# yixuan/LBFGSpp

Hardware: NVIDIA B200
Metric: lbfgs_iterations_per_sec (higher is better)
Workload: dtype f64

## Files before the change

### lbfgspp_b200/csrc/device_utils.cuh

```cuda
#pragma once

#include <cuda_runtime.h>
#include <stdint.h>

namespace lb {

constexpr int kThreads = 256;
constexpr int kMaxRed = 8;
constexpr int kMaxBlocks = 148 * 8;

template <class T> struct Pack { T v[4]; };

enum class Hint { Stream, Keep, Plain };

template <Hint H> __device__ __forceinline__ Pack<double> ld_pack(const double* p)
{
    Pack<double> r;
    if (H == Hint::Stream)
        asm("ld.global.L1::no_allocate.L2::evict_first.v4.f64 {%0,%1,%2,%3}, [%4];"
                     : "=d"(r.v[0]), "=d"(r.v[1]), "=d"(r.v[2]), "=d"(r.v[3]) : "l"(p));
    else if (H == Hint::Keep)
        asm("ld.global.L1::no_allocate.L2::evict_last.v4.f64 {%0,%1,%2,%3}, [%4];"
                     : "=d"(r.v[0]), "=d"(r.v[1]), "=d"(r.v[2]), "=d"(r.v[3]) : "l"(p));
    else
        asm("ld.global.v4.f64 {%0,%1,%2,%3}, [%4];"
                     : "=d"(r.v[0]), "=d"(r.v[1]), "=d"(r.v[2]), "=d"(r.v[3]) : "l"(p));
    return r;
}
template <Hint H> __device__ __forceinline__ void st_pack(double* p, const Pack<double>& r)
{
    if (H == Hint::Stream)
        asm volatile("st.global.L1::no_allocate.L2::evict_first.v4.f64 [%0], {%1,%2,%3,%4};"
                     :: "l"(p), "d"(r.v[0]), "d"(r.v[1]), "d"(r.v[2]), "d"(r.v[3]) : "memory");
    else if (H == Hint::Keep)
        asm volatile("st.global.L1::no_allocate.L2::evict_last.v4.f64 [%0], {%1,%2,%3,%4};"
                     :: "l"(p), "d"(r.v[0]), "d"(r.v[1]), "d"(r.v[2]), "d"(r.v[3]) : "memory");
    else
        asm volatile("st.global.v4.f64 [%0], {%1,%2,%3,%4};"
                     :: "l"(p), "d"(r.v[0]), "d"(r.v[1]), "d"(r.v[2]), "d"(r.v[3]) : "memory");
}
template <Hint H> __device__ __forceinline__ Pack<float> ld_pack(const float* p)
{
    Pack<float> r;
    if (H == Hint::Plain)
        asm("ld.global.v4.f32 {%0,%1,%2,%3}, [%4];"
                     : "=f"(r.v[0]), "=f"(r.v[1]), "=f"(r.v[2]), "=f"(r.v[3]) : "l"(p));
    else
        asm("ld.global.L1::no_allocate.v4.f32 {%0,%1,%2,%3}, [%4];"
                     : "=f"(r.v[0]), "=f"(r.v[1]), "=f"(r.v[2]), "=f"(r.v[3]) : "l"(p));
    return r;
}
template <Hint H> __device__ __forceinline__ void st_pack(float* p, const Pack<float>& r)
{
    asm volatile("st.global.v4.f32 [%0], {%1,%2,%3,%4};"
                 :: "l"(p), "f"(r.v[0]), "f"(r.v[1]), "f"(r.v[2]), "f"(r.v[3]) : "memory");
}

template <class T> __host__ __device__ __forceinline__ bool pack_aligned(const void* p)
{
    return (reinterpret_cast<uintptr_t>(p) & (sizeof(T) * 4 - 1)) == 0;
}

template <class T, Hint H, bool VEC> __device__ __forceinline__ Pack<T> load4(const T* base, int64_t i0, int cnt)
{
    if (VEC && cnt == 4) return ld_pack<H>(base + i0);
    Pack<T> r;
#pragma unroll
    for (int k = 0; k < 4; k++) r.v[k] = (k < cnt) ? base[i0 + k] : T(0);
    return r;
}
template <class T, Hint H, bool VEC> __device__ __forceinline__ void store4(T* base, int64_t i0, int cnt, const Pack<T>& r)
{
    if (VEC && cnt == 4) { st_pack<H>(base + i0, r); return; }
#pragma unroll
    for (int k = 0; k < 4; k++)
        if (k < cnt) base[i0 + k] = r.v[k];
}

constexpr int kXMaxRanks = 8;
constexpr int kXRing = 4;
constexpr int kXMaxVals = 4608;
constexpr int kMailVals = 384;

struct XInbox
{
    double vals[kXRing][kXMaxRanks][kXMaxVals];
    unsigned long long flag[kXRing][kXMaxRanks];
    unsigned long long ll[kXRing][kXMaxRanks][kXMaxVals][2];
};

__device__ __forceinline__ void ll_push(unsigned long long* dst2, double v, unsigned tag)
{
    const unsigned long long bits = (unsigned long long)__double_as_longlong(v);
    const unsigned long long w0 = (bits & 0xffffffffull) | ((unsigned long long)tag << 32);
    const unsigned long long w1 = (bits >> 32) | ((unsigned long long)tag << 32);
    asm volatile("st.volatile.global.v2.u64 [%0], {%1, %2};" :: "l"(dst2), "l"(w0), "l"(w1) : "memory");
}
template <class GiveUp> __device__ __forceinline__ bool ll_pull(const unsigned long long* src2, unsigned tag, double& v, GiveUp give_up)
{
    for (;;)
    {
        unsigned long long w0, w1;
        asm volatile("ld.volatile.global.v2.u64 {%0, %1}, [%2];" : "=l"(w0), "=l"(w1) : "l"(src2) : "memory");
        if ((unsigned)(w0 >> 32) == tag && (unsigned)(w1 >> 32) == tag)
        {
            v = __longlong_as_double((long long)((w0 & 0xffffffffull) | (w1 << 32)));
            return true;
        }
        if (give_up()) return false;
    }
}

struct XComm
{
    XInbox* inbox[kXMaxRanks];
    int rank, nranks;
};

struct ReduceBuf
{
    double* partials;
    unsigned* ticket;
    double* result;
    const XComm* xc;
    unsigned long long epoch;
    double* mail_vals;
    unsigned long long* mail_word;
    unsigned long long mail_seq;
    const int* mail_flag_src;
    int* mail_flag_dst;
};

__device__ __forceinline__ void st_release_sys(unsigned long long* p, unsigned long long v)
{
    asm volatile("st.release.sys.global.u64 [%0], %1;" :: "l"(p), "l"(v) : "memory");
}
__device__ __forceinline__ unsigned long long ld_acquire_sys(const unsigned long long* p)
{
    unsigned long long v;
    asm volatile("ld.acquire.sys.global.u64 %0, [%1];" : "=l"(v) : "l"(p) : "memory");
    return v;
}
__device__ __forceinline__ double ld_volatile_f64(const double* p)
{
    double v;
    asm volatile("ld.volatile.global.f64 %0, [%1];" : "=d"(v) : "l"(p) : "memory");
    return v;
}

__device__ __forceinline__ void xrank_allreduce(double* result, int nv, const XComm* xc, unsigned long long epoch)
{
    const int tid = threadIdx.x, nt = blockDim.x;
    const int slot = (int)(epoch % kXRing), me = xc->rank, R = xc->nranks;
    __syncthreads();
    for (int i = tid; i < nv * R; i += nt)
    {
        const int dst = i / nv, k = i % nv;
        xc->inbox[dst]->vals[slot][me][k] = result[k];
    }
    __threadfence_system();
    __syncthreads();
    if (tid < R) st_release_sys(&xc->inbox[tid]->flag[slot][me], epoch);
    if (tid < R)
    {
        const unsigned long long* f = &xc->inbox[me]->flag[slot][tid];
        while (ld_acquire_sys(f) != epoch) {}
    }
    __syncthreads();
    for (int k = tid; k < nv; k += nt)
    {
        double t = 0.0;
        for (int r = 0; r < R; r++) t += ld_volatile_f64(&xc->inbox[me]->vals[slot][r][k]);
        result[k] = t;
    }
    __threadfence();
    __syncthreads();
}

__device__ __forceinline__ void deliver_to_host(const ReduceBuf& rb, int nv)
{
    if (rb.mail_seq == 0ull) return;
    for (int k = threadIdx.x; k < nv; k += blockDim.x) rb.mail_vals[k] = rb.result[k];
    if (threadIdx.x == 0 && rb.mail_flag_src) *rb.mail_flag_dst = *rb.mail_flag_src;
    __threadfence_system();
    __syncthreads();
    if (threadIdx.x == 0) st_release_sys(rb.mail_word, rb.mail_seq);
}


__device__ __forceinline__ double warp_sum(double v)
{
#pragma unroll
    for (int o = 16; o > 0; o >>= 1) v += __shfl_xor_sync(0xffffffffu, v, o);
    return v;
}

template <int NV> __device__ __forceinline__ bool grid_reduce(const double (&acc)[NV], const ReduceBuf& rb)
{
    __shared__ double s_part[NV][kThreads / 32];
    __shared__ bool s_last;
    const int lane = threadIdx.x & 31, warp = threadIdx.x >> 5;
#pragma unroll
    for (int k = 0; k < NV; k++)
    {
        const double w = warp_sum(acc[k]);
        if (lane == 0) s_part[k][warp] = w;
    }
    __syncthreads();
    if (threadIdx.x < NV)
    {
        double t = 0.0;
#pragma unroll
        for (int w = 0; w < kThreads / 32; w++) t += s_part[threadIdx.x][w];
        rb.partials[blockIdx.x * kMaxRed + threadIdx.x] = t;
    }
    __threadfence();
    __syncthreads();
    if (threadIdx.x == 0)
    {
        const unsigned t = atomicAdd(rb.ticket, 1u);
        s_last = (t == gridDim.x - 1);
    }
    __syncthreads();
    if (!s_last) return false;
    __threadfence();
    double mine[NV];
#pragma unroll
    for (int k = 0; k < NV; k++) mine[k] = 0.0;
    for (unsigned b = threadIdx.x; b < gridDim.x; b += kThreads)
#pragma unroll
        for (int k = 0; k < NV; k++) mine[k] += __ldcg(&rb.partials[b * kMaxRed + k]);
    __syncthreads();
#pragma unroll
    for (int k = 0; k < NV; k++)
    {
        const double w = warp_sum(mine[k]);
        if (lane == 0) s_part[k][warp] = w;
    }
    __syncthreads();
    if (threadIdx.x < NV)
    {
        double t = 0.0;
#pragma unroll
        for (int w = 0; w < kThreads / 32; w++) t += s_part[threadIdx.x][w];
        rb.result[threadIdx.x] = t;
    }
    if (threadIdx.x == 0) *rb.ticket = 0u;
    __threadfence();
    __syncthreads();
    if (rb.xc != nullptr) xrank_allreduce(rb.result, NV, rb.xc, rb.epoch);
    deliver_to_host(rb, NV);
    return true;
}

}
```

### lbfgspp_b200/csrc/persist.cuh

```cuda
#pragma once

#include "../../include/LBFGSpp/LineSearchCore.h"

namespace lb {

constexpr int kMaxPast = 64;
constexpr int kPThreads = kGramMaxThreads;
constexpr int kPWarps = kPThreads / 32;
constexpr int kPStageBytes = kGramStages * 4 * kGramTE * 8;
constexpr int kPMaxStages = 4;
constexpr int kPCache = 4;

enum { POP_IDLE = 0, POP_FIRST = 1, POP_TRIAL = 2, POP_DOTS_FORM = 3, POP_DOTS_PLAIN = 4, POP_COMBINE = 5, POP_COMBINE_TRIAL = 6, POP_RESTORE = 7,
       POP_MATERIALIZE = 8 };
constexpr int kPOps = 10;
constexpr int kPGramScratch = 1024;

template <class T> struct PHist
{
    T* H;
    int bt_log, M;
    int64_t bstride;
    __device__ __forceinline__ int BT() const { return 1 << bt_log; }
    __device__ __forceinline__ T* s_at(int slot, int64_t i) const { return H + (i >> bt_log) * bstride + ((int64_t)slot << (bt_log + 1)) + (i & (BT() - 1)); }
    __device__ __forceinline__ T* y_at(int slot, int64_t i) const { return s_at(slot, i) + BT(); }
};

template <class T> struct PState
{
    T *x, *xp, *g, *gp, *drt, *x_lo, *g_lo;
    PHist<T> hist;
    T *ys, *alpha, *theta;
    T *SY[2], *YY[2], *SS[2];
    const T *data0, *data1;
    double* raw;
    double* halo;
    int head, ncorr, M, m, gram_cur, pending;
    int op, c_round;
    T epsilon, epsilon_rel, delta, max_step, eps_gate;
    int past, max_iterations, ls_kind, fuse_first_trial;
    LBFGSpp::LineSearchOptions<T> ls_opt;
    LBFGSpp::BacktrackingCore<T> bt;
    LBFGSpp::BracketingCore<T> br;
    LBFGSpp::NocedalWrightCore<T> nw;
    LBFGSpp::MoreThuenteCore<T> mt;
    int have_lo;
    T lo_gg, lo_xx, start_gg, start_xx;
    int first_store;
    int adaptive_first_store;
    int lo_virtual;
    T lo_step;
    int after_materialize;
    T fx, dg, gg, xx, gnorm, step;
    int k;
    long long nfev;
    int status;
    int finished;
    int niter;
    T fx_hist[kMaxPast];
    double* trace;
    long long trace_cap;
    long long rounds;
};

template <class T> struct alignas(128) PRound
{
    T *x, *xp, *g, *gp, *drt;
    T step;
    int op, c_round, head, pending, gram_cur, store_first;
};

struct alignas(128) PCtl
{
    unsigned arrive;
    unsigned pad0[31];
    unsigned release;
    unsigned pad1[31];
    int abort;
    int nactive;
    unsigned long long epoch;
    unsigned long long rounds;
    long long cyc_op[kPOps];
    long long cyc_sync;
    long long cyc_wait_all;
    long long cyc_exchange;
    unsigned long long n_op[kPOps];
    double words_op[kPOps];
};
constexpr unsigned kPStopBit = 0x80000000u;

template <class T> struct PArgs
{
    PState<T>* probs;
    PRound<T>* rounds;
    int B;
    PCtl* ctl;
    double* partials;
    int pstride;
    int64_t n;
    int grain;
    const XComm* xc;
    int64_t index_offset, n_global;
    long long wait_cycles;
    int tune;
};

template <class V> __device__ __forceinline__ V ldv(const V* p) { return *reinterpret_cast<const volatile V*>(p); }

template <class T> __device__ __forceinline__ T& ls_step_ref(PState<T>* st)
{
    switch (st->ls_kind)
    {
    case 0: return st->bt.step;
    case 1: return st->br.step;
    case 2: return st->nw.step;
    default: return st->mt.step;
    }
}
template <class T> __device__ __forceinline__ int ls_init(PState<T>* st, T fx, T dg, T step, T step_max)
{
    switch (st->ls_kind)
    {
    case 0: return st->bt.init(st->ls_opt, fx, dg, step, step_max);
    case 1: return st->br.init(st->ls_opt, fx, dg, step, step_max);
    case 2: return st->nw.init(st->ls_opt, fx, dg, step, step_max);
    default: return st->mt.init(st->ls_opt, fx, dg, step, step_max);
    }
}
template <class T> __device__ __forceinline__ int ls_advance(PState<T>* st, T fx, T dg, bool& keep)
{
    switch (st->ls_kind)
    {
    case 0: return st->bt.advance(fx, dg, keep);
    case 1: return st->br.advance(fx, dg, keep);
    case 2: return st->nw.advance(fx, dg, keep);
    default: return st->mt.advance(fx, dg, keep);
    }
}
template <class T> __device__ __forceinline__ void ls_best(PState<T>* st, T& fx, T& dg)
{
    switch (st->ls_kind)
    {
    case 0: fx = st->bt.best_fx; dg = st->bt.best_dg; break;
    case 1: fx = st->br.best_fx; dg = st->br.best_dg; break;
    case 2: fx = st->nw.best_fx; dg = st->nw.best_dg; break;
    default: fx = st->mt.best_fx; dg = st->mt.best_dg; break;
    }
}
template <class P> __device__ __forceinline__ void dswap(P& a, P& b) { P t = a; a = b; b = t; }
__device__ __forceinline__ int slot_by_age(int head, int M, int age) { return ((head - 1 - age) % M + M) % M; }

template <class T, class OBJ> struct PObjMaker;
template <class T> struct PObjMaker<T, RosenbrockPaired<T> >
{ static __device__ RosenbrockPaired<T> make(const PArgs<T>& a, const T*, const T*, const double*) { return RosenbrockPaired<T>{a.n}; } };
template <class T> struct PObjMaker<T, QuadShift<T> >
{ static __device__ QuadShift<T> make(const PArgs<T>& a, const T*, const T*, const double*) { return QuadShift<T>{a.n, a.index_offset}; } };
template <class T> struct PObjMaker<T, RosenbrockChained<T> >
{ static __device__ RosenbrockChained<T> make(const PArgs<T>& a, const T*, const T*, const double* halo)
  { return RosenbrockChained<T>{a.n, a.index_offset, a.n_global, halo}; } };
template <class T> struct PObjMaker<T, QuadTridiag<T> >
{ static __device__ QuadTridiag<T> make(const PArgs<T>& a, const T* d0, const T* d1, const double* halo)
  { return QuadTridiag<T>{a.n, d0, d1, a.index_offset, a.n_global, halo}; } };

struct PShared
{
    uint64_t full_bar[kPMaxStages];
    double red[kPWarps][3 * kGramVals];
    double coef[2 * kMaxM + 2];
    const void* vecs[2 * kMaxM + 2];
    unsigned char slots[kMaxM];
    unsigned char slotid[kMaxM];
    double margin[2][2 * kMaxM + 2];
    double carry[2];
    unsigned char ops[4096];
};

struct Own
{
    int64_t n;
    int G, cta;
    int64_t c0, c1;
    __device__ __forceinline__ Own(int64_t n_, int G_, int cta_, int grain) : n(n_), G(G_), cta(cta_)
    {
        const int64_t units = (n + grain - 1) / grain;
        const int64_t K = units < G ? units : G;
        if (cta >= K) { c0 = c1 = 0; return; }
        c0 = ((units * cta) / K) * grain;
        c1 = ((units * (cta + 1)) / K) * grain;
        if (c1 > n) c1 = n;
    }
    __device__ __forceinline__ int64_t ntiles(int TE) const { return (c1 - c0 + TE - 1) / TE; }
    __device__ __forceinline__ int64_t start(int64_t t, int TE) const { return c0 + t * TE; }
    __device__ __forceinline__ int len(int64_t t, int TE) const
    {
        const int64_t rest = c1 - start(t, TE);
        return rest <= 0 ? 0 : (rest < TE ? (int)rest : TE);
    }
};

template <int NV> __device__ __forceinline__ void block_sums(const double (&acc)[NV], PShared& sh, double* dst, int G)
{
    const int lane = threadIdx.x & 31, warp = threadIdx.x >> 5;
    __syncthreads();
#pragma unroll
    for (int k = 0; k < NV; k++)
    {
        const double w = warp_sum(acc[k]);
        if (lane == 0) sh.red[warp][k] = w;
    }
    __syncthreads();
    if (threadIdx.x < NV)
    {
        double t = 0.0;
#pragma unroll
        for (int w = 0; w < kPWarps; w++) t += sh.red[w][threadIdx.x];
        dst[(size_t)threadIdx.x * G] = t;
    }
}

template <class T, class OBJ, int MODE>
__device__ __forceinline__ void p_trial(const OBJ& obj, const Own& own, const T* __restrict__ xp, const T* __restrict__ d, T step,
                                        T* __restrict__ x, T* __restrict__ g, T* __restrict__ dout, PShared& sh, double* dst, int G, int tune)
{
    T acc[4] = {T(0), T(0), T(0), T(0)};
    const int64_t n = own.n;
    const int64_t p1 = (own.c1 + 3) >> 2;
    const bool evict_first = (tune & 4) != 0;
    auto body = [&](int64_t q) {
        const int64_t i0 = q << 2;
        const int cnt = (n - i0 >= 4) ? 4 : int(n - i0);
        T xv[4], dv[4] = {T(0), T(0), T(0), T(0)}, gv[4];
        T xl = T(0), xr = T(0);
        if (MODE == 1)
        {
            const Pack<T> px = load4<T, Hint::Stream, true>(xp, i0, cnt), pd = load4<T, Hint::Stream, true>(d, i0, cnt);
#pragma unroll
            for (int k = 0; k < 4; k++) { dv[k] = pd.v[k]; xv[k] = px.v[k] + step * pd.v[k]; }
            if constexpr (OBJ::kHalo)
            {
                if (i0 > 0) xl = __ldcg(xp + i0 - 1) + step * __ldcg(d + i0 - 1);
                else if (obj.halo && obj.gofs > 0) xl = T(ldv(obj.halo + kHaloLeftA)) + step * T(ldv(obj.halo + kHaloLeftB));
                if (i0 + 4 < n) xr = __ldcg(xp + i0 + 4) + step * __ldcg(d + i0 + 4);
                else if (obj.halo && i0 + 4 == n && obj.gofs + n < obj.n_glob) xr = T(ldv(obj.halo + kHaloRightA)) + step * T(ldv(obj.halo + kHaloRightB));
            }
        }
        else
        {
            const Pack<T> px = load4<T, Hint::Stream, true>(x, i0, cnt);
#pragma unroll
            for (int k = 0; k < 4; k++) xv[k] = px.v[k];
            if constexpr (OBJ::kHalo)
            {
                if (i0 > 0) xl = __ldcg(x + i0 - 1);
                else if (obj.halo && obj.gofs > 0) xl = T(ldv(obj.halo + kHaloLeftA));
                if (i0 + 4 < n) xr = __ldcg(x + i0 + 4);
                else if (obj.halo && i0 + 4 == n && obj.gofs + n < obj.n_glob) xr = T(ldv(obj.halo + kHaloRightA));
            }
        }
        acc[0] += obj.eval(i0, cnt, xv, xl, xr, gv);
        Pack<T> pg, po;
#pragma unroll
        for (int k = 0; k < 4; k++)
        {
            acc[1] += gv[k] * dv[k];
            acc[2] += gv[k] * gv[k];
            acc[3] += (k < cnt) ? xv[k] * xv[k] : T(0);
            pg.v[k] = gv[k];
            po.v[k] = (MODE == 1) ? xv[k] : T(-1) * gv[k];
        }
        T* const out0 = (MODE == 1) ? x : dout;
        if (evict_first) { store4<T, Hint::Stream, true>(out0, i0, cnt, po); store4<T, Hint::Stream, true>(g, i0, cnt, pg); }
        else { store4<T, Hint::Plain, true>(out0, i0, cnt, po); store4<T, Hint::Plain, true>(g, i0, cnt, pg); }
    };
#pragma unroll 2
    for (int64_t q = (own.c0 >> 2) + threadIdx.x; q < p1; q += kPThreads) body(q);
    const double dacc[4] = {(double)acc[0], (double)acc[1], (double)acc[2], (double)acc[3]};
    block_sums<4>(dacc, sh, dst, G);
}

constexpr int kTrialTE = 2016;

template <class T, class OBJ, int MODE>
__device__ __forceinline__ void p_trial_halo(const OBJ& obj, const Own& own, const T* __restrict__ xp, const T* __restrict__ d, T step,
                                             T* __restrict__ x, T* __restrict__ g, T* __restrict__ dout, T* tiles, PShared& sh, unsigned& phase_bits,
                                             double* dst, int G)
{
    constexpr int NIN = (MODE == 1) ? 2 : 1;
    constexpr int DV = OBJ::kDataVectors;
    constexpr int NVEC = NIN + DV;
    constexpr int PAD = 16 / (int)sizeof(T);
    constexpr int TS = kTrialTE + 2 * PAD;
    constexpr int STAGES_MAX = kPStageBytes / (NVEC * TS * (int)sizeof(T));
    constexpr int STAGES = STAGES_MAX > kPMaxStages ? kPMaxStages : STAGES_MAX;
    const int tid = threadIdx.x, lane = tid & 31;
    uint64_t* full_bar = sh.full_bar;
    const T* in0 = (MODE == 1) ? xp : x;
    const int64_t n = own.n;
    const int64_t ntl = own.ntiles(kTrialTE);
    const int64_t n_pad = (n + 31) & ~int64_t(31);

    auto stage_tile = [&](int64_t t, int stage) {
        if (tid != 0) return;
        T* dstt = tiles + (size_t)stage * NVEC * TS;
        const int64_t e0 = own.start(t, kTrialTE);
        const int64_t lo = e0 >= PAD ? e0 - PAD : 0;
        int64_t hi = e0 + ((own.len(t, kTrialTE) + 31) & ~31) + PAD;
        if (hi > n_pad) hi = n_pad;
        const unsigned bytes = (unsigned)(hi - lo) * (unsigned)sizeof(T);
        const int shift = (int)(lo - (e0 - PAD));
        asm volatile("fence.proxy.async.shared::cta;" ::: "memory");
        mbar_expect_tx(&full_bar[stage], bytes * NVEC);
        tma_load_1d(dstt + shift, in0 + lo, bytes, &full_bar[stage]);
        if (MODE == 1) tma_load_1d(dstt + TS + shift, d + lo, bytes, &full_bar[stage]);
        if constexpr (DV == 2)
        {
            tma_load_1d(dstt + (size_t)NIN * TS + shift, obj.diag + lo, bytes, &full_bar[stage]);
            tma_load_1d(dstt + (size_t)(NIN + 1) * TS + shift, obj.rhs + lo, bytes, &full_bar[stage]);
        }
    };

    T acc[4] = {T(0), T(0), T(0), T(0)};
    __syncthreads();
    int64_t next_tile = 0;
    for (int s = 0; s < STAGES; s++, next_tile++)
        if (next_tile < ntl) stage_tile(next_tile, s);
    int stage = 0;
    for (int64_t t = 0; t < ntl; t++)
    {
        mbar_wait(&full_bar[stage], (phase_bits >> stage) & 1u);
        phase_bits ^= (1u << stage);
        const T* ta = tiles + (size_t)stage * NVEC * TS + PAD;
        const T* tb = ta + TS;
        const int64_t e0 = own.start(t, kTrialTE);
        const int len = own.len(t, kTrialTE);
        for (int off = tid * 4; off < len; off += kPThreads * 4)
        {
            const int64_t i0 = e0 + off;
            const int cnt = (len - off >= 4) ? 4 : (len - off);
            T xv[4], dv[4] = {T(0), T(0), T(0), T(0)}, gv[4];
            T xl = T(0), xr = T(0);
            const Pack<T> pa = lds_pack(ta + off, lane);
            if (MODE == 1)
            {
                const Pack<T> pb = lds_pack(tb + off, lane);
#pragma unroll
                for (int k = 0; k < 4; k++) { dv[k] = (k < cnt) ? pb.v[k] : T(0); xv[k] = (k < cnt) ? pa.v[k] + step * pb.v[k] : T(0); }
                if (i0 > 0) xl = ta[off - 1] + step * tb[off - 1];
                else if (obj.halo && obj.gofs > 0) xl = T(ldv(obj.halo + kHaloLeftA)) + step * T(ldv(obj.halo + kHaloLeftB));
                if (i0 + 4 < n) xr = ta[off + 4] + step * tb[off + 4];
                else if (obj.halo && i0 + 4 == n && obj.gofs + n < obj.n_glob) xr = T(ldv(obj.halo + kHaloRightA)) + step * T(ldv(obj.halo + kHaloRightB));
            }
            else
            {
#pragma unroll
                for (int k = 0; k < 4; k++) xv[k] = (k < cnt) ? pa.v[k] : T(0);
                if (i0 > 0) xl = ta[off - 1];
                else if (obj.halo && obj.gofs > 0) xl = T(ldv(obj.halo + kHaloLeftA));
                if (i0 + 4 < n) xr = ta[off + 4];
                else if (obj.halo && i0 + 4 == n && obj.gofs + n < obj.n_glob) xr = T(ldv(obj.halo + kHaloRightA));
            }
            if constexpr (DV == 2) acc[0] += obj.staged(ta + (size_t)NIN * TS, ta + (size_t)(NIN + 1) * TS, e0).eval(i0, cnt, xv, xl, xr, gv);
            else acc[0] += obj.eval(i0, cnt, xv, xl, xr, gv);
            Pack<T> pg, po;
#pragma unroll
            for (int k = 0; k < 4; k++)
            {
                acc[1] += gv[k] * dv[k];
                acc[2] += gv[k] * gv[k];
                acc[3] += (k < cnt) ? xv[k] * xv[k] : T(0);
                pg.v[k] = gv[k];
                po.v[k] = (MODE == 1) ? xv[k] : T(-1) * gv[k];
            }
            if (MODE == 1) store4<T, Hint::Plain, true>(x, i0, cnt, po);
            else store4<T, Hint::Plain, true>(dout, i0, cnt, po);
            store4<T, Hint::Plain, true>(g, i0, cnt, pg);
        }
        asm volatile("fence.proxy.async.shared::cta;" ::: "memory");
        __syncthreads();
        if (next_tile < ntl) stage_tile(next_tile, stage);
        next_tile++;
        stage = (stage + 1 == STAGES) ? 0 : stage + 1;
    }
    const double dacc[4] = {(double)acc[0], (double)acc[1], (double)acc[2], (double)acc[3]};
    block_sums<4>(dacc, sh, dst, G);
}

template <class T>
__device__ __forceinline__ void p_restore(const Own& own, const T* __restrict__ xp, const T* __restrict__ gp, T* __restrict__ x, T* __restrict__ g)
{
    const int64_t n = own.n;
    const int64_t p1 = (own.c1 + 3) >> 2;
    for (int64_t q = (own.c0 >> 2) + threadIdx.x; q < p1; q += kPThreads)
    {
        const int64_t i0 = q << 2;
        const int cnt = (n - i0 >= 4) ? 4 : int(n - i0);
        store4<T, Hint::Plain, true>(x, i0, cnt, load4<T, Hint::Stream, true>(xp, i0, cnt));
        store4<T, Hint::Plain, true>(g, i0, cnt, load4<T, Hint::Stream, true>(gp, i0, cnt));
    }
}

struct SlotRuns
{
    int a0, a1, b0, b1;
    __device__ __forceinline__ SlotRuns(int end, int cnt, int M)
    {
        if (cnt <= end) { a0 = end - cnt; a1 = end; b0 = b1 = 0; }
        else { a0 = 0; a1 = end; b0 = M - (cnt - end); b1 = M; }
    }
    __device__ __forceinline__ int row_of(int slot) const { return (slot >= a0 && slot < a1) ? slot - a0 : (a1 - a0) + (slot - b0); }
};

template <class T> struct alignas(16) Unit { T v[16 / sizeof(T)]; };
template <class T> __device__ __forceinline__ Unit<T> lds_unit(const T* p)
{
    Unit<T> u;
    *reinterpret_cast<float4*>(u.v) = *reinterpret_cast<const float4*>(p);
    return u;
}
template <class T> __device__ __forceinline__ void st_unit(T* base, int64_t i0, int cnt, const Unit<T>& u)
{
    constexpr int EPT = 16 / (int)sizeof(T);
    if (cnt >= EPT) { *reinterpret_cast<float4*>(base + i0) = *reinterpret_cast<const float4*>(u.v); return; }
#pragma unroll
    for (int k = 0; k < EPT; k++)
        if (k < cnt) base[i0 + k] = u.v[k];
}
template <class T> __device__ __forceinline__ void mask_unit(Unit<T>& u, int cnt)
{
#pragma unroll
    for (int k = 0; k < 16 / (int)sizeof(T); k++) u.v[k] = (k < cnt) ? u.v[k] : T(0);
}

template <class T>
__device__ __forceinline__ void stage_tiled(T* dstt, int TE, int nrhs, int64_t e0, int len, const PHist<T>& h, const SlotRuns& runs, PShared& sh,
                                            uint64_t* bar)
{
    const int tid = threadIdx.x;
    if (tid >= 32) return;
    const unsigned rbytes = (unsigned)((len + 31) & ~31) * (unsigned)sizeof(T);
    const unsigned abytes = (unsigned)(runs.a1 - runs.a0) * 2u * (unsigned)TE * (unsigned)sizeof(T);
    const unsigned bbytes = (unsigned)(runs.b1 - runs.b0) * 2u * (unsigned)TE * (unsigned)sizeof(T);
    if (tid == 0)
    {
        asm volatile("fence.proxy.async.shared::cta;" ::: "memory");
        mbar_expect_tx(bar, rbytes * (unsigned)nrhs + abytes + bbytes);
    }
    __syncwarp();
    const T* blk = h.H + (e0 >> h.bt_log) * h.bstride;
    if (tid < nrhs) tma_load_1d(dstt + (size_t)tid * TE, static_cast<const T*>(sh.vecs[tid]) + e0, rbytes, bar);
    else if (tid == nrhs && abytes) tma_load_1d(dstt + (size_t)nrhs * TE, blk + (size_t)runs.a0 * 2 * TE, abytes, bar);
    else if (tid == nrhs + 1 && bbytes) tma_load_1d(dstt + (size_t)(nrhs + 2 * (runs.a1 - runs.a0)) * TE, blk + (size_t)runs.b0 * 2 * TE, bbytes, bar);
}

template <class T> struct PDots
{
    int64_t n;
    PHist<T> h;
    int c;
    int end, cnt_old;
    int new_slot, split, cols_per_round;
};

template <class T, int ROUNDS, bool FORM>
__device__ __forceinline__ void p_dots(const PDots<T>& a, const Own& own, T* tiles, PShared& sh, unsigned& phase_bits, double* dst, int G)
{
    constexpr int EPT = 16 / (int)sizeof(T);
    constexpr int NRHS = FORM ? 4 : 1;
    const int tid = threadIdx.x, lane = tid & 31, warp = tid >> 5;
    const int TE = a.h.BT();
    const int my_col = warp / a.split, my_part = warp % a.split;
    const int upp = (TE / EPT) / a.split;
    const SlotRuns runs(a.end, a.cnt_old, a.h.M);
    const int nrows = NRHS + 2 * a.cnt_old;
    int stages = (int)((size_t)kPStageBytes / ((size_t)nrows * TE * sizeof(T)));
    stages = stages > kPMaxStages ? kPMaxStages : stages;
    const int64_t ntl = own.ntiles(TE);
    uint64_t* full_bar = sh.full_bar;

    T acc[ROUNDS][kGramVals];
#pragma unroll
    for (int r = 0; r < ROUNDS; r++)
#pragma unroll
        for (int k = 0; k < kGramVals; k++) acc[r][k] = T(0);

    __syncthreads();
    int64_t next_tile = 0;
    for (int s = 0; s < stages; s++, next_tile++)
        if (next_tile < ntl) stage_tiled<T>(tiles + (size_t)s * nrows * TE, TE, NRHS, own.start(next_tile, TE), own.len(next_tile, TE), a.h, runs, sh, &full_bar[s]);
    int stage = 0;
    for (int64_t t = 0; t < ntl; t++)
    {
        mbar_wait(&full_bar[stage], (phase_bits >> stage) & 1u);
        phase_bits ^= (1u << stage);
        const T* base = tiles + (size_t)stage * nrows * TE;
        const T* hist = base + (size_t)NRHS * TE;
        const int64_t e0 = own.start(t, TE);
        const int len = own.len(t, TE);
#pragma unroll
        for (int r = 0; r < ROUNDS; r++)
        {
            const int j = r * a.cols_per_round + my_col;
            if (my_col < a.cols_per_round && j < a.c)
            {
                const bool is_new = FORM && j == 0;
                const T* srow = hist + (size_t)2 * (is_new ? 0 : sh.slots[j]) * TE;
                const T* yrow = srow + TE;
                T* s_new = a.h.s_at(a.new_slot < 0 ? 0 : a.new_slot, e0);
                for (int u = my_part * upp + lane; u < (my_part + 1) * upp; u += 32)
                {
                    const int off = u * EPT;
                    const int cnt = len - off;
                    if (cnt <= 0) break;
                    Unit<T> ug = lds_unit<T>(base + off), us, uy, usn, uyn;
                    if constexpr (FORM)
                    {
                        const Unit<T> ux = lds_unit<T>(base + TE + off), ugp = lds_unit<T>(base + 2 * TE + off), uxp = lds_unit<T>(base + 3 * TE + off);
#pragma unroll
                        for (int k = 0; k < EPT; k++) { usn.v[k] = ux.v[k] - uxp.v[k]; uyn.v[k] = ug.v[k] - ugp.v[k]; }
                        if (cnt < EPT) { mask_unit(usn, cnt); mask_unit(uyn, cnt); }
                    }
                    bool loaded = false;
                    if constexpr (FORM)
                    {
                        if (is_new)
                        {
                            us = usn; uy = uyn;
                            st_unit<T>(s_new, off, cnt, usn);
                            st_unit<T>(s_new + TE, off, cnt, uyn);
                            loaded = true;
                        }
                    }
                    if (!loaded) { us = lds_unit<T>(srow + off); uy = lds_unit<T>(yrow + off); }
                    if (cnt < EPT) { mask_unit(ug, cnt); mask_unit(us, cnt); mask_unit(uy, cnt); }
#pragma unroll
                    for (int k = 0; k < EPT; k++)
                    {
                        acc[r][0] += us.v[k] * ug.v[k];
                        acc[r][1] += uy.v[k] * ug.v[k];
                    }
                    if constexpr (FORM)
                    {
#pragma unroll
                        for (int k = 0; k < EPT; k++)
                        {
                            acc[r][2] += us.v[k] * uyn.v[k];
                            acc[r][3] += uy.v[k] * uyn.v[k];
                            acc[r][4] += uy.v[k] * usn.v[k];
                            acc[r][5] += us.v[k] * usn.v[k];
                        }
                    }
                }
            }
        }
        asm volatile("fence.proxy.async.shared::cta;" ::: "memory");
        __syncthreads();
        if (next_tile < ntl) stage_tiled<T>(tiles + (size_t)stage * nrows * TE, TE, NRHS, own.start(next_tile, TE), own.len(next_tile, TE), a.h, runs, sh, &full_bar[stage]);
        next_tile++;
        stage = (stage + 1 == stages) ? 0 : stage + 1;
    }

#pragma unroll
    for (int r = 0; r < ROUNDS; r++)
#pragma unroll
        for (int k = 0; k < kGramVals; k++)
        {
            const double w = warp_sum((double)acc[r][k]);
            if (lane == 0) sh.red[warp][r * kGramVals + k] = w;
        }
    __syncthreads();
    const int nvals = a.c * kGramVals;
    for (int idx = tid; idx < nvals; idx += kPThreads)
    {
        const int j = idx / kGramVals, k = idx % kGramVals;
        const int r = j / a.cols_per_round, col = j % a.cols_per_round;
        double t = 0.0;
        for (int p = 0; p < a.split; p++) t += sh.red[col * a.split + p][r * kGramVals + k];
        dst[(size_t)idx * G] = t;
    }
}

__device__ __forceinline__ void dots_geometry(int c, int units, int& split, int& cols_per_round)
{
    split = 8;
    while (split > 1 && (c * split > kGramMaxWarps || units / split < 32)) split >>= 1;
    cols_per_round = c < kGramMaxWarps / split ? c : kGramMaxWarps / split;
}

template <class T, class OBJ, bool FUSE, bool HALO, class Between>
__device__ __forceinline__ void p_combine(const OBJ& obj, const Own& own, const PHist<T>& h, int c, int end, T* tiles, T* __restrict__ res,
                                          T* __restrict__ x1_out, T* __restrict__ g1_out, PShared& sh, unsigned& phase_bits, double* dst, int G,
                                          Between between)
{
    constexpr int EPT = 16 / (int)sizeof(T);
    constexpr int DV = HALO ? OBJ::kDataVectors : 0;
    constexpr int NRHS = (FUSE ? 2 : 1) + DV;
    constexpr int PAD = EPT;
    const int tid = threadIdx.x, lane = tid & 31, warp = tid >> 5;
    const int TE = h.BT();
    const SlotRuns runs(end, c, h.M);
    const int nrows = NRHS + 2 * c;
    const size_t stage_elems = (size_t)nrows * TE + (HALO ? 2 * PAD : 0);
    int stages = (int)((size_t)kPStageBytes / (stage_elems * sizeof(T)));
    stages = stages > kPMaxStages ? kPMaxStages : stages;
    const int64_t n = own.n;
    const int64_t ntl = own.ntiles(TE);
    const T* s_coef = reinterpret_cast<const T*>(sh.coef);
    uint64_t* full_bar = sh.full_bar;
    auto stage_one = [&](int64_t t, int s) {
        T* dstt = tiles + (size_t)s * stage_elems;
        if (!HALO) { stage_tiled<T>(dstt, TE, NRHS, own.start(t, TE), own.len(t, TE), h, runs, sh, &full_bar[s]); return; }
        if (tid >= 32) return;
        const int64_t e0 = own.start(t, TE);
        const int len = own.len(t, TE);
        const unsigned rbytes = (unsigned)((len + 31) & ~31) * (unsigned)sizeof(T);
        const unsigned abytes = (unsigned)(runs.a1 - runs.a0) * 2u * (unsigned)TE * (unsigned)sizeof(T);
        const unsigned bbytes = (unsigned)(runs.b1 - runs.b0) * 2u * (unsigned)TE * (unsigned)sizeof(T);
        if (tid == 0)
        {
            asm volatile("fence.proxy.async.shared::cta;" ::: "memory");
            mbar_expect_tx(&full_bar[s], rbytes * (unsigned)NRHS + abytes + bbytes);
        }
        __syncwarp();
        const T* blk = h.H + (e0 >> h.bt_log) * h.bstride;
        T* hist = dstt + (size_t)NRHS * TE + 2 * PAD;
        if (tid == 0) tma_load_1d(dstt, static_cast<const T*>(sh.vecs[0]) + e0, rbytes, &full_bar[s]);
        else if (tid == 1) tma_load_1d(dstt + TE + PAD, static_cast<const T*>(sh.vecs[1]) + e0, rbytes, &full_bar[s]);
        else if (tid == 2 && abytes) tma_load_1d(hist, blk + (size_t)runs.a0 * 2 * TE, abytes, &full_bar[s]);
        else if (tid == 3 && bbytes) tma_load_1d(hist + (size_t)2 * (runs.a1 - runs.a0) * TE, blk + (size_t)runs.b0 * 2 * TE, bbytes, &full_bar[s]);
        else if (tid >= 4 && tid < 4 + DV) tma_load_1d(dstt + (size_t)(tid - 2) * TE + 2 * PAD, static_cast<const T*>(sh.vecs[tid - 2]) + e0, rbytes, &full_bar[s]);
    };

    T acc[5] = {T(0), T(0), T(0), T(0), T(0)};
    T pre[5] = {T(0), T(0), T(0), T(0), T(0)};
    __syncthreads();
    int64_t next_tile = 0;
    for (int s = 0; s < stages; s++, next_tile++)
        if (next_tile < ntl) stage_one(next_tile, s);
    between();
    const T cv = s_coef[0];
    int stage = 0;
    for (int64_t t = 0; t < ntl; t++)
    {
        mbar_wait(&full_bar[stage], (phase_bits >> stage) & 1u);
        phase_bits ^= (1u << stage);
        T* base = tiles + (size_t)stage * stage_elems;
        T* xrow = base + TE + (HALO ? PAD : 0);
        const T* hist = base + (size_t)NRHS * TE + (HALO ? 2 * PAD : 0);
        const int len = own.len(t, TE);
        const int64_t e0 = own.start(t, TE);
        auto direction = [&](int off, T (&r)[EPT], Unit<T>& uv) {
            uv = lds_unit<T>(base + off);
#pragma unroll
            for (int k = 0; k < EPT; k++) r[k] = cv * uv.v[k];
#pragma unroll 8
            for (int j = 0; j < c; j++)
            {
                const Unit<T> uy = lds_unit<T>(hist + ((size_t)2 * sh.slots[j] + 1) * TE + off);
                const T cy = s_coef[1 + j];
#pragma unroll
                for (int k = 0; k < EPT; k++) r[k] += cy * uy.v[k];
            }
#pragma unroll 8
            for (int j = c - 1; j >= 0; j--)
            {
                const Unit<T> us = lds_unit<T>(hist + (size_t)2 * sh.slots[j] * TE + off);
                const T cs = s_coef[1 + c + j];
#pragma unroll
                for (int k = 0; k < EPT; k++) r[k] += cs * us.v[k];
            }
        };
        if constexpr (!HALO)
        {
            for (int off = tid * EPT; off < len; off += kPThreads * EPT)
            {
                const int cnt = (len - off >= EPT) ? EPT : (len - off);
                T r[EPT];
                Unit<T> uv;
                direction(off, r, uv);
                Unit<T> out;
#pragma unroll
                for (int k = 0; k < EPT; k++)
                {
                    out.v[k] = r[k];
                    acc[0] += (k < cnt) ? uv.v[k] * r[k] : T(0);
                }
                const int64_t i0 = e0 + off;
                st_unit<T>(res, i0, cnt, out);
                if constexpr (FUSE)
                {
                    const Unit<T> ux = lds_unit<T>(xrow + off);
                    T xv[4] = {T(0), T(0), T(0), T(0)}, gv[4];
#pragma unroll
                    for (int k = 0; k < EPT; k++) xv[k] = (k < cnt) ? ux.v[k] + T(1) * r[k] : T(0);
                    acc[1] += obj.eval(i0, cnt, xv, T(0), T(0), gv);
                    Unit<T> ug, uo;
#pragma unroll
                    for (int k = 0; k < EPT; k++)
                    {
                        acc[2] += (k < cnt) ? gv[k] * r[k] : T(0);
                        acc[3] += (k < cnt) ? gv[k] * gv[k] : T(0);
                        acc[4] += (k < cnt) ? xv[k] * xv[k] : T(0);
                        ug.v[k] = gv[k];
                        uo.v[k] = xv[k];
                    }
                    if (x1_out != nullptr)
                    {
                        st_unit<T>(x1_out, i0, cnt, uo);
                        st_unit<T>(g1_out, i0, cnt, ug);
                    }
                }
            }
        }
        else
        {
            const int off = tid * EPT;
            const bool mine = off < len;
            const int64_t i0 = e0 + off;
            const int cnt = mine ? ((len - off >= EPT) ? EPT : (len - off)) : 0;
            T r[EPT];
#pragma unroll
            for (int k = 0; k < EPT; k++) r[k] = T(0);
            if (mine)
            {
                Unit<T> uv;
                direction(off, r, uv);
                Unit<T> out;
#pragma unroll
                for (int k = 0; k < EPT; k++)
                {
                    out.v[k] = r[k];
                    acc[0] += (k < cnt) ? uv.v[k] * r[k] : T(0);
                }
                st_unit<T>(res, i0, cnt, out);
                const Unit<T> ux = lds_unit<T>(xrow + off);
                Unit<T> u1;
#pragma unroll
                for (int k = 0; k < EPT; k++) u1.v[k] = (k < cnt) ? ux.v[k] + T(1) * r[k] : T(0);
                *reinterpret_cast<float4*>(xrow + off) = *reinterpret_cast<const float4*>(u1.v);
            }
            if (warp == kPWarps - 2 && lane == 0 && t > 0) xrow[-1] = *reinterpret_cast<const T*>(&sh.carry[(t - 1) & 1]);
            if (warp >= kPWarps - 2 && (warp == kPWarps - 1 || t == 0))
            {
                const bool left = warp == kPWarps - 2;
                const int64_t im = left ? e0 - 1 : e0 + len;
                T* scratch = reinterpret_cast<T*>(sh.margin[left ? 0 : 1]);
                auto fetch = [&](int64_t i, T (&dstv)[5]) {
#pragma unroll
                    for (int w = 0; w < 5; w++)
                    {
                        const int q = lane + 32 * w;
                        T val = T(0);
                        if (i >= 0 && i < n && q < 2 * c + 2)
                        {
                            if (q == 0) val = __ldcg(static_cast<const T*>(sh.vecs[0]) + i);
                            else if (q == 1) val = __ldcg(static_cast<const T*>(sh.vecs[1]) + i);
                            else if (q < 2 + c) val = __ldcg(h.y_at(sh.slotid[q - 2], i));
                            else val = __ldcg(h.s_at(sh.slotid[q - 2 - c], i));
                        }
                        dstv[w] = val;
                    }
                };
                if (left || t == 0) fetch(im, pre);
                if (im >= 0 && im < n)
                {
#pragma unroll
                    for (int w = 0; w < 5; w++)
                    {
                        const int q = lane + 32 * w;
                        if (q < 2 * c + 2)
                            scratch[q] = (q == 0) ? cv * pre[w] : (q == 1) ? pre[w] : (q < 2 + c) ? s_coef[1 + (q - 2)] * pre[w] : s_coef[1 + c + (q - 2 - c)] * pre[w];
                    }
                    __syncwarp();
                    if (lane == 0)
                    {
                        T rm = scratch[0];
                        for (int j = 0; j < c; j++) rm += scratch[2 + j];
                        for (int j = c - 1; j >= 0; j--) rm += scratch[2 + c + j];
                        xrow[left ? -1 : len] = scratch[1] + T(1) * rm;
                    }
                }
                if (!left && t + 1 < ntl) fetch(own.start(t + 1, TE) + own.len(t + 1, TE), pre);
            }
            if (mine && off + EPT >= len) *reinterpret_cast<T*>(&sh.carry[t & 1]) = xrow[len - 1];
            __syncthreads();
            if (mine)
            {
                T xv[4] = {T(0), T(0), T(0), T(0)}, gv[4];
                const Unit<T> u1 = lds_unit<T>(xrow + off);
#pragma unroll
                for (int k = 0; k < EPT; k++) xv[k] = u1.v[k];
                const T xl = (i0 > 0) ? xrow[off - 1] : T(0);
                const T right = (i0 + EPT < n) ? xrow[off + EPT] : T(0);
                T xr = T(0);
                if (EPT < 4) xv[EPT < 4 ? EPT : 3] = right; else xr = right;
                if constexpr (DV == 2) acc[1] += obj.staged(base + 2 * (size_t)TE + 2 * PAD, base + 3 * (size_t)TE + 2 * PAD, e0).eval(i0, cnt, xv, xl, xr, gv);
                else acc[1] += obj.eval(i0, cnt, xv, xl, xr, gv);
                Unit<T> ug, uo;
#pragma unroll
                for (int k = 0; k < EPT; k++)
                {
                    acc[2] += (k < cnt) ? gv[k] * r[k] : T(0);
                    acc[3] += (k < cnt) ? gv[k] * gv[k] : T(0);
                    acc[4] += (k < cnt) ? xv[k] * xv[k] : T(0);
                    ug.v[k] = gv[k];
                    uo.v[k] = xv[k];
                }
                if (x1_out != nullptr)
                {
                    st_unit<T>(x1_out, i0, cnt, uo);
                    st_unit<T>(g1_out, i0, cnt, ug);
                }
            }
        }
        asm volatile("fence.proxy.async.shared::cta;" ::: "memory");
        __syncthreads();
        if (next_tile < ntl) stage_one(next_tile, stage);
        next_tile++;
        stage = (stage + 1 == stages) ? 0 : stage + 1;
    }
    if (FUSE)
    {
        const double dacc[5] = {(double)acc[0], (double)acc[1], (double)acc[2], (double)acc[3], (double)acc[4]};
        block_sums<5>(dacc, sh, dst, G);
    }
    else
    {
        const double dacc[1] = {(double)acc[0]};
        block_sums<1>(dacc, sh, dst, G);
    }
}

constexpr long long kPWaitCycles = 6000000000ll;

__device__ __forceinline__ unsigned ld_acquire_gpu_u32(const unsigned* p)
{
    unsigned v;
    asm volatile("ld.acquire.gpu.global.u32 %0, [%1];" : "=r"(v) : "l"(p) : "memory");
    return v;
}
__device__ __forceinline__ void st_release_gpu_u32(unsigned* p, unsigned v)
{
    asm volatile("st.release.gpu.global.u32 [%0], %1;" :: "l"(p), "r"(v) : "memory");
}

template <class T> __device__ __forceinline__ void record_eval(PState<T>* st, T fx)
{
    if (st->trace && st->nfev < st->trace_cap) st->trace[st->nfev] = (double)fx;
    st->nfev++;
}
template <class T> __device__ __forceinline__ void finish(PState<T>* st, int niter, int status = 0)
{
    st->finished = 1;
    st->niter = niter;
    if (status) st->status = status;
    st->op = POP_IDLE;
}

template <class T> __device__ __forceinline__ bool converged_after_search(PState<T>* st)
{
    const int k = st->k;
    st->gnorm = sqrt(st->gg);
    if (st->gnorm <= st->epsilon || st->gnorm <= st->epsilon_rel * sqrt(st->xx)) { finish(st, k); return true; }
    if (st->past > 0)
    {
        const T fxd = st->fx_hist[k % st->past];
        const T fx = st->fx;
        const T afx = fx < T(0) ? -fx : fx, afxd = fxd < T(0) ? -fxd : fxd;
        T big = afx < afxd ? afxd : afx;
        big = big < T(1) ? T(1) : big;
        const T diff = (fxd - fx) < T(0) ? -(fxd - fx) : (fxd - fx);
        if (k >= st->past && diff <= st->delta * big) { finish(st, k); return true; }
        st->fx_hist[k % st->past] = fx;
    }
    if (st->max_iterations != 0 && k >= st->max_iterations) { finish(st, k); return true; }
    return false;
}

template <class T> __device__ __forceinline__ void after_search(PState<T>* st)
{
    if (converged_after_search(st)) return;
    st->op = POP_DOTS_FORM;
    st->c_round = st->ncorr < st->m ? st->ncorr + 1 : st->m;
}

template <class T> __device__ __forceinline__ void digest_trial(PState<T>* st, T fx, T dg, T gg, T xx, bool is_first, bool is_virtual)
{
    record_eval(st, fx);
    bool keep = false;
    const T step_tried = ls_step_ref(st);
    const int rc = ls_advance(st, fx, dg, keep);
    if (is_first && st->adaptive_first_store) st->first_store = (rc == LBFGSpp::LSC_ACCEPT) ? 1 : 0;
    if (keep)
    {
        if (is_virtual) { st->lo_virtual = 1; st->lo_step = step_tried; }
        else
        {
            dswap(st->x, st->x_lo);
            dswap(st->g, st->g_lo);
            st->lo_virtual = 0;
        }
        st->have_lo = 1;
        st->lo_gg = gg;
        st->lo_xx = xx;
    }
    if (rc == LBFGSpp::LSC_EVALUATE) { st->op = POP_TRIAL; st->step = ls_step_ref(st); return; }
    if (rc == LBFGSpp::LSC_ACCEPT)
    {
        st->fx = fx; st->dg = dg; st->gg = gg; st->xx = xx;
        if (is_virtual) { st->op = POP_MATERIALIZE; st->step = step_tried; st->after_materialize = 1; return; }
    }
    else if (rc == LBFGSpp::LSC_TAKE_BEST)
    {
        T bf, bd;
        ls_best(st, bf, bd);
        st->fx = bf;
        st->dg = bd;
        if (st->have_lo)
        {
            st->gg = st->lo_gg;
            st->xx = st->lo_xx;
            if (st->lo_virtual) { st->op = POP_MATERIALIZE; st->step = st->lo_step; st->after_materialize = 2; return; }
            dswap(st->x, st->x_lo);
            dswap(st->g, st->g_lo);
        }
        else
        {
            st->gg = st->start_gg;
            st->xx = st->start_xx;
            st->op = POP_RESTORE;
            return;
        }
    }
    else { finish(st, st->k, rc); return; }
    after_search(st);
}

template <class T> __device__ __forceinline__ bool begin_search(PState<T>* st, T step)
{
    const int rc = ls_init(st, st->fx, st->dg, step, st->max_step);
    if (rc != 0) { finish(st, st->k, rc); return false; }
    dswap(st->xp, st->x);
    dswap(st->gp, st->g);
    st->have_lo = 0;
    st->lo_virtual = 0;
    st->start_gg = st->gg;
    st->start_xx = st->xx;
    st->op = POP_TRIAL;
    st->step = ls_step_ref(st);
    return true;
}

template <class T> __device__ void advance_problem(PState<T>* st, const double* vals)
{
    st->rounds++;
    switch (st->op)
    {
    case POP_FIRST:
    {
        const T fx = (T)vals[0], gg = (T)vals[2], xx = (T)vals[3];
        st->nfev = 0;
        record_eval(st, fx);
        st->fx = fx; st->gg = gg; st->xx = xx;
        st->k = 1;
        if (st->past > 0) st->fx_hist[0] = fx;
        st->gnorm = sqrt(gg);
        if (st->gnorm <= st->epsilon || st->gnorm <= st->epsilon_rel * sqrt(xx)) { finish(st, 1); return; }
        st->dg = -gg;
        begin_search(st, T(1) / st->gnorm);
        return;
    }
    case POP_TRIAL:
        digest_trial(st, (T)vals[0], (T)vals[1], (T)vals[2], (T)vals[3], false, false);
        return;
    case POP_RESTORE:
    case POP_MATERIALIZE:
        after_search(st);
        return;
    case POP_DOTS_FORM:
    {
        const T sy = (T)vals[2], yy = (T)vals[3];
        if (sy > st->eps_gate * yy)
        {
            st->ys[st->head] = sy;
            *st->theta = yy / sy;
            st->pending = st->head;
            st->head = (st->head + 1) % st->M;
            st->ncorr = st->c_round;
            st->op = st->fuse_first_trial ? POP_COMBINE_TRIAL : POP_COMBINE;
        }
        else if (st->ncorr > 0) { st->op = POP_DOTS_PLAIN; st->c_round = st->ncorr; }
        else { st->op = st->fuse_first_trial ? POP_COMBINE_TRIAL : POP_COMBINE; st->c_round = 0; }
        return;
    }
    case POP_DOTS_PLAIN:
        st->op = st->fuse_first_trial ? POP_COMBINE_TRIAL : POP_COMBINE;
        return;
    case POP_COMBINE:
    case POP_COMBINE_TRIAL:
    {
        const bool fused = st->op == POP_COMBINE_TRIAL;
        const bool stored = st->first_store != 0;
        if (st->pending >= 0) { st->gram_cur = 1 - st->gram_cur; st->pending = -1; }
        st->dg = (T)vals[0];
        st->k += 1;
        if (!begin_search(st, T(1))) return;
        if (fused && ls_step_ref(st) == T(1)) digest_trial(st, (T)vals[1], (T)vals[2], (T)vals[3], (T)vals[4], true, !stored);
        return;
    }
    default: return;
    }
}

__device__ __forceinline__ double words_of(int op, int c, int data_vectors, int store_first)
{
    switch (op)
    {
    case POP_FIRST: return 3.0 + data_vectors;
    case POP_TRIAL: case POP_MATERIALIZE: return 4.0 + data_vectors;
    case POP_RESTORE: return 4.0;
    case POP_DOTS_FORM: return 2.0 * c + 4.0;
    case POP_DOTS_PLAIN: return 2.0 * c + 1.0;
    case POP_COMBINE: return 2.0 * c + 2.0;
    case POP_COMBINE_TRIAL: return 2.0 * c + 3.0 + (store_first ? 2.0 : 0.0) + data_vectors;
    default: return 0.0;
    }
}

template <class T> __device__ __forceinline__ int nvals_of(const PState<T>* st)
{
    switch (st->op)
    {
    case POP_FIRST: case POP_TRIAL: case POP_MATERIALIZE: return 4;
    case POP_DOTS_FORM: case POP_DOTS_PLAIN: return st->c_round * kGramVals;
    case POP_COMBINE: return 1;
    case POP_COMBINE_TRIAL: return 5;
    default: return 0;
    }
}

template <class T, bool HALO>
__device__ int leader_round(const PArgs<T>& a, int G, PShared& sh, PState<T>* cache)
{
    const int tid = threadIdx.x;
    auto state_of = [&](int b) -> PState<T>* { return b < kPCache ? cache + b : a.probs + b; };
    for (int b = 0; b < a.B; b++)
    {
        PState<T>* st = state_of(b);
        const int op = st->op;
        if (op == POP_IDLE) continue;
        const int nv = nvals_of(st);
        const double* part = a.partials + (size_t)b * a.pstride * G;
        for (int v0 = 0; v0 < nv; v0 += kPThreads / 16)
        {
            const int v = v0 + tid / 16, sub = tid & 15;
            double t = 0.0;
            if (v < nv)
                for (int cta = sub; cta < G; cta += 16) t += __ldcg(part + (size_t)v * G + cta);
            t += __shfl_xor_sync(0xffffffffu, t, 8);
            t += __shfl_xor_sync(0xffffffffu, t, 4);
            t += __shfl_xor_sync(0xffffffffu, t, 2);
            t += __shfl_xor_sync(0xffffffffu, t, 1);
            if (v < nv && sub == 0) st->raw[v] = t;
        }
    }
    __syncthreads();
    if (a.xc != nullptr)
    {
        const long long t_x0 = clock64();
        const XComm* xc = a.xc;
        const int me = xc->rank, R = xc->nranks;
        const unsigned long long epoch = a.ctl->epoch + 1ull;
        const int slot = (int)(epoch % kXRing);
        const unsigned tag = (unsigned)epoch;
        auto give_up = [&]() {
            if (clock64() - t_x0 > 4 * a.wait_cycles || ldv(&a.ctl->abort)) { a.ctl->abort = 1; return true; }
            return false;
        };
        int ofs = 0;
        for (int b = 0; b < a.B; b++)
        {
            PState<T>* st = state_of(b);
            const int op = st->op;
            if (op == POP_IDLE) continue;
            const int nv = nvals_of(st);
            for (int r = tid; r < R * nv; r += kPThreads)
                ll_push(xc->inbox[r / nv]->ll[slot][me][ofs + r % nv], st->raw[r % nv], tag);
            ofs += nv;
            if (HALO)
            {
                if (tid < 4 * R)
                {
                    const int k = tid & 3;
                    const T* src = (k & 1) ? st->drt : st->x;
                    const double val = (double)__ldcg(src + ((k & 2) ? a.n - 1 : 0));
                    ll_push(xc->inbox[tid >> 2]->ll[slot][me][ofs + k], val, tag);
                }
                ofs += 4;
            }
        }
        __syncthreads();
        ofs = 0;
        for (int b = 0; b < a.B; b++)
        {
            PState<T>* st = state_of(b);
            const int op = st->op;
            if (op == POP_IDLE) continue;
            const int nv = nvals_of(st);
            for (int k = tid; k < nv; k += kPThreads)
            {
                double t = 0.0;
                for (int r = 0; r < R; r++)
                {
                    double v = 0.0;
                    ll_pull(xc->inbox[me]->ll[slot][r][ofs + k], tag, v, give_up);
                    t += v;
                }
                st->raw[k] = t;
            }
            ofs += nv;
            if (HALO)
            {
                if ((op == POP_FIRST || op == POP_COMBINE || op == POP_COMBINE_TRIAL) && tid < 8)
                {
                    const int side = tid >> 2, k = tid & 3;
                    const int nb = side == 0 ? me - 1 : me + 1;
                    double v = 0.0;
                    if (nb >= 0 && nb < R) ll_pull(xc->inbox[me]->ll[slot][nb][ofs + k], tag, v, give_up);
                    st->halo[4 + 4 * side + k] = v;
                }
                ofs += 4;
            }
        }
        __syncthreads();
        if (tid == 0) { a.ctl->epoch = epoch; a.ctl->cyc_exchange += clock64() - t_x0; }
    }
    int still = 0;
    for (int b0 = 0; b0 < a.B; b0 += kPThreads)
    {
        const int b = b0 + tid;
        int running = 0;
        if (b < a.B && state_of(b)->op != POP_IDLE)
        {
            PState<T>* st = state_of(b);
            advance_problem(st, st->raw);
            PRound<T>* rd = a.rounds + b;
            rd->x = st->x; rd->xp = st->xp; rd->g = st->g; rd->gp = st->gp; rd->drt = st->drt;
            rd->step = st->step;
            rd->c_round = st->c_round; rd->head = st->head; rd->pending = st->pending; rd->gram_cur = st->gram_cur;
            rd->store_first = st->first_store;
            rd->op = st->op;
            running = st->op != POP_IDLE;
        }
        still += __syncthreads_count(running);
    }
    if (tid == 0) { a.ctl->nactive = still; a.ctl->rounds++; }
    return still;
}

template <class T> __device__ void leader_halo_prelude(const PArgs<T>& a)
{
    const int tid = threadIdx.x;
    const XComm* xc = a.xc;
    const int me = xc->rank, R = xc->nranks;
    const unsigned long long epoch = a.ctl->epoch + 1ull;
    const int slot = (int)(epoch % kXRing);
    const unsigned tag = (unsigned)epoch;
    const long long t_x0 = clock64();
    auto give_up = [&]() {
        if (clock64() - t_x0 > 4 * a.wait_cycles || ldv(&a.ctl->abort)) { a.ctl->abort = 1; return true; }
        return false;
    };
    for (int b = 0; b < a.B; b++)
    {
        PState<T>* st = a.probs + b;
        if (tid < 4 * R)
        {
            const int k = tid & 3;
            const double val = (k & 1) ? 0.0 : (double)__ldcg(st->x + ((k & 2) ? a.n - 1 : 0));
            ll_push(xc->inbox[tid >> 2]->ll[slot][me][4 * b + k], val, tag);
        }
    }
    for (int b = 0; b < a.B; b++)
    {
        PState<T>* st = a.probs + b;
        if (tid < 8)
        {
            const int side = tid >> 2, k = tid & 3;
            const int nb = side == 0 ? me - 1 : me + 1;
            double v = 0.0;
            if (nb >= 0 && nb < R) ll_pull(xc->inbox[me]->ll[slot][nb][4 * b + k], tag, v, give_up);
            st->halo[4 + 4 * side + k] = v;
        }
    }
    __syncthreads();
    if (tid == 0) a.ctl->epoch = epoch;
}

template <class T, class OBJ, int ROUNDS>
__global__ void __launch_bounds__(kPThreads, 1) k_persist(PArgs<T> a)
{
    extern __shared__ __align__(128) unsigned char p_smem[];
    T* tiles = reinterpret_cast<T*>(p_smem);
    __shared__ PShared sh;
    const int tid = threadIdx.x, G = gridDim.x, cta = blockIdx.x;
    const Own own(a.n, G, cta, a.grain);
    if (tid == 0)
    {
        for (int s = 0; s < kPMaxStages; s++) mbar_init(&sh.full_bar[s], 1);
        asm volatile("fence.mbarrier_init.release.cluster;" ::: "memory");
    }
    __syncthreads();
    unsigned phase_bits = 0;
    unsigned episode = 0;
    constexpr bool HALO = OBJ::kHalo;
    constexpr int kDataVectors = OBJ::kDataVectors;
    long long t_last = clock64(), t_arrive = 0;
    int acct_bucket = 0;
    double acct_words = 0.0;
    __shared__ unsigned s_release;
    __shared__ __align__(16) double s_gram[kPGramScratch];
    __shared__ PState<T> s_state[kPCache];
    const int ncache = a.B < kPCache ? a.B : kPCache;
    if (cta == 0)
    {
        const unsigned* src = reinterpret_cast<const unsigned*>(a.probs);
        unsigned* dstw = reinterpret_cast<unsigned*>(s_state);
        for (int w = tid; w < (int)(sizeof(PState<T>) / 4) * ncache; w += kPThreads) dstw[w] = src[w];
        __syncthreads();
    }

    auto grid_barrier = [&](auto leader_work) -> bool {
        episode++;
        asm volatile("fence.proxy.async;" ::: "memory");
        if (HALO) __threadfence();
        __syncthreads();
        if (tid == 0) { __threadfence(); atomicAdd(&a.ctl->arrive, 1u); }
        if (cta == 0)
        {
            if (tid == 0)
            {
                const long long t_start = clock64();
                t_arrive = t_start;
                while (ld_acquire_gpu_u32(&a.ctl->arrive) != episode * (unsigned)G)
                    if (clock64() - t_start > a.wait_cycles || ldv(&a.ctl->abort)) { a.ctl->abort = 1; break; }
                a.ctl->cyc_wait_all += clock64() - t_start;
            }
            __syncthreads();
            const bool stop = leader_work();
            __syncthreads();
            if (tid == 0)
            {
                const long long now = clock64();
                a.ctl->cyc_op[acct_bucket] += now - t_last;
                a.ctl->cyc_sync += now - t_arrive;
                a.ctl->n_op[acct_bucket] += 1ull;
                a.ctl->words_op[acct_bucket] += acct_words;
                t_last = now;
                st_release_gpu_u32(&a.ctl->release, episode | (stop ? kPStopBit : 0u));
            }
        }
        if (tid == 0)
        {
            const long long t_start = clock64();
            unsigned v;
            while (((v = ld_acquire_gpu_u32(&a.ctl->release)) & ~kPStopBit) < episode)
                if (clock64() - t_start > 6 * a.wait_cycles || ldv(&a.ctl->abort)) { a.ctl->abort = 1; v = kPStopBit; break; }
            s_release = v;
        }
        __syncthreads();
        return (s_release & kPStopBit) != 0u;
    };

    if (HALO && a.xc != nullptr)
        if (grid_barrier([&]() { leader_halo_prelude<T>(a); return ldv(&a.ctl->abort) != 0; })) return;

    for (;;)
    {
        if (a.B > 1)
        {
            for (int b = tid; b < a.B; b += kPThreads) sh.ops[b] = (unsigned char)ldv(&a.rounds[b].op);
            __syncthreads();
        }
        acct_bucket = -1;
        acct_words = 0.0;
        for (int b = 0; b < a.B; b++)
        {
            const PRound<T>* rd = a.rounds + b;
            if (a.B > 1 && sh.ops[b] == POP_IDLE) continue;
            const int op = (a.B > 1) ? (int)sh.ops[b] : ldv(&rd->op);
            const PState<T>* st = a.probs + b;
            T* const vx = ldv(&rd->x); T* const vxp = ldv(&rd->xp); T* const vg = ldv(&rd->g); T* const vgp = ldv(&rd->gp); T* const vd = ldv(&rd->drt);
            const T step = ldv(&rd->step);
            const int c_round = ldv(&rd->c_round), head = ldv(&rd->head), pending = ldv(&rd->pending), gram_cur = ldv(&rd->gram_cur);
            const int store_first = ldv(&rd->store_first);
            if (op == POP_IDLE) continue;
            acct_bucket = (acct_bucket == -1 || acct_bucket == op) ? op : 0;
            acct_words += words_of(op, c_round, kDataVectors, store_first);
            double* dst = a.partials + (size_t)b * a.pstride * G + cta;
            const OBJ obj = PObjMaker<T, OBJ>::make(a, st->data0, st->data1, (HALO && a.xc != nullptr) ? st->halo : nullptr);
            switch (op)
            {
            case POP_FIRST:
                if constexpr (HALO) p_trial_halo<T, OBJ, 0>(obj, own, nullptr, nullptr, T(0), vx, vg, vd, tiles, sh, phase_bits, dst, G);
                else p_trial<T, OBJ, 0>(obj, own, nullptr, nullptr, T(0), vx, vg, vd, sh, dst, G, a.tune);
                break;
            case POP_TRIAL:
            case POP_MATERIALIZE:
                if constexpr (HALO) p_trial_halo<T, OBJ, 1>(obj, own, vxp, vd, step, vx, vg, nullptr, tiles, sh, phase_bits, dst, G);
                else p_trial<T, OBJ, 1>(obj, own, vxp, vd, step, vx, vg, nullptr, sh, dst, G, a.tune);
                break;
            case POP_RESTORE:
                p_restore<T>(own, vxp, vgp, vx, vg);
                break;
            case POP_DOTS_FORM:
            case POP_DOTS_PLAIN:
            {
                const bool form = op == POP_DOTS_FORM;
                PDots<T> d;
                d.n = a.n; d.h = st->hist; d.c = c_round;
                d.end = head;
                d.cnt_old = form ? c_round - 1 : c_round;
                d.new_slot = form ? head : -1;
                dots_geometry(d.c, d.h.BT() / (16 / (int)sizeof(T)), d.split, d.cols_per_round);
                __syncthreads();
                {
                    const SlotRuns runs(d.end, d.cnt_old, d.h.M);
                    if (tid < d.c && !(form && tid == 0))
                        sh.slots[tid] = (unsigned char)runs.row_of(slot_by_age(head, d.h.M, form ? tid - 1 : tid));
                    if (tid == 0) { sh.vecs[0] = vg; sh.vecs[1] = vx; sh.vecs[2] = vgp; sh.vecs[3] = vxp; }
                }
                if (form) p_dots<T, ROUNDS, true>(d, own, tiles, sh, phase_bits, dst, G);
                else p_dots<T, ROUNDS, false>(d, own, tiles, sh, phase_bits, dst, G);
                break;
            }
            case POP_COMBINE:
            case POP_COMBINE_TRIAL:
            {
                GramSolveArgs<T> g;
                g.c = c_round;
                g.M = st->hist.M; g.new_slot = pending; g.with_v = 1; g.a = T(-1);
                g.raw = st->raw;
                const int in = gram_cur, out = (g.new_slot >= 0) ? 1 - in : in;
                g.SY_in = st->SY[in]; g.YY_in = st->YY[in]; g.SS_in = st->SS[in];
                g.SY_out = st->SY[out]; g.YY_out = st->YY[out]; g.SS_out = st->SS[out];
                g.ys = st->ys; g.alpha = st->alpha; g.theta = st->theta;
                g.ov_slot = -1; g.ov_theta_on = 0;
                for (int age = 0; age < g.c; age++) g.slots[age] = (unsigned char)slot_by_age(head, g.M, age);
                __syncthreads();
                const bool fuse = op == POP_COMBINE_TRIAL;
                {
                    const SlotRuns runs(head, g.c, g.M);
                    for (int j = tid; j < g.c; j += kPThreads)
                    {
                        sh.slots[j] = (unsigned char)runs.row_of(g.slots[j]);
                        sh.slotid[j] = g.slots[j];
                    }
                    if (tid == 0) { sh.vecs[0] = vg; sh.vecs[1] = vx; sh.vecs[2] = st->data0; sh.vecs[3] = st->data1; }
                }
                const bool own_scratch = gram_solve_smem_elems(g.c) * sizeof(T) <= sizeof(s_gram);
                auto solve_into = [&](T* scratch) {
                    gram_solve_in_smem<T>(g, scratch, cta == 0);
                    const T* s_coef = scratch + 2 * g.c * g.c;
                    T* keep = reinterpret_cast<T*>(sh.coef);
                    for (int q = tid; q < 2 * g.c + 1; q += kPThreads) keep[q] = s_coef[q];
                    __syncthreads();
                };
                if (!own_scratch) solve_into(tiles);
                auto between = [&]() { if (own_scratch) solve_into(reinterpret_cast<T*>(s_gram)); };
                if (fuse) p_combine<T, OBJ, true, OBJ::kHalo>(obj, own, st->hist, g.c, head, tiles, vd, store_first ? vxp : nullptr, store_first ? vgp : nullptr, sh, phase_bits, dst, G, between);
                else p_combine<T, OBJ, false, false>(obj, own, st->hist, g.c, head, tiles, vd, nullptr, nullptr, sh, phase_bits, dst, G, between);
                break;
            }
            default: break;
            }
        }
        if (acct_bucket < 0) acct_bucket = 0;
        if (grid_barrier([&]() { return leader_round<T, HALO>(a, G, sh, s_state) == 0 || ldv(&a.ctl->abort) != 0; })) break;
    }
    if (cta == 0)
    {
        __syncthreads();
        const unsigned* src = reinterpret_cast<const unsigned*>(s_state);
        unsigned* dstw = reinterpret_cast<unsigned*>(a.probs);
        for (int w = tid; w < (int)(sizeof(PState<T>) / 4) * ncache; w += kPThreads) dstw[w] = src[w];
    }
}

}
```

### lbfgspp_b200/csrc/persist_host.cuh

```cuda
#pragma once

struct lbfgs_b200_solver
{
    lbfgs_b200_ctx* ctx = nullptr;
    int64_t n = 0;
    int m = 0, elem = 8, B = 1;
    void* d_hist = nullptr;
    int bt_log = 9, M = 0;
    size_t hist_elems = 0;
    void* d_small = nullptr;
    size_t small_elems = 0;
    std::vector<int> ring_head, ring_ncorr, ring_gram_cur;
    std::vector<lbfgs_b200_hist*> exported;
    std::vector<char> export_fresh;
    void* vec_slab = nullptr;
    size_t vec_elems = 0;
    void* d_state = nullptr;
    void* d_rounds = nullptr;
    lb::PCtl* d_ctl = nullptr;
    double* d_partials = nullptr;
    double* d_raw = nullptr;
    double* d_halo = nullptr;
    int pstride = 0;
    double* d_trace = nullptr;
    long long trace_cap = 0;
    std::vector<void*> final_g, final_x;
    std::vector<unsigned char> h_state;
    std::vector<unsigned char> h_rounds;
    cudaEvent_t ev0 = nullptr, ev1 = nullptr;
    float last_kernel_ms = 0.f;
    lb::PCtl last_ctl{};
};

template <class T> static void* persist_kernel_for(int objective, int rounds)
{
    using namespace lb;
#define LB_PK(OBJ) (rounds <= 1 ? (void*)k_persist<T, OBJ, 1> : rounds == 2 ? (void*)k_persist<T, OBJ, 2> : (void*)k_persist<T, OBJ, 3>)
    switch (objective)
    {
    case LBFGS_B200_OBJ_ROSENBROCK_PAIRED: return LB_PK(RosenbrockPaired<T>);
    case LBFGS_B200_OBJ_QUAD_SHIFT: return LB_PK(QuadShift<T>);
    case LBFGS_B200_OBJ_ROSENBROCK_CHAINED: return LB_PK(RosenbrockChained<T>);
    case LBFGS_B200_OBJ_QUAD_TRIDIAG: return LB_PK(QuadTridiag<T>);
    }
#undef LB_PK
    return nullptr;
}

template <class T>
static lbfgs_b200_status solver_minimize(lbfgs_b200_solver* s, int objective, const T* data0, const T* data1, int64_t ldd, const lbfgs_b200_param* prm,
                                         int ls_kind, T* x_inout, int64_t ldx, double* trace_host, long long trace_cap, lbfgs_b200_outcome* outs)
{
    using namespace lb;
    lbfgs_b200_ctx* ctx = s->ctx;
    const int B = s->B;
    REQUIRE(ctx, s->elem == (int)sizeof(T), "solver element size mismatch");
    REQUIRE(ctx, prm && outs && x_inout, "solver_minimize: NULL argument");
    REQUIRE(ctx, prm->m == s->m, "solver was created for m = %d, called with m = %d", s->m, prm->m);
    REQUIRE(ctx, ls_kind >= 0 && ls_kind <= 3, "unknown line search %d", ls_kind);
    REQUIRE(ctx, prm->past <= kMaxPast, "past > %d is not supported by the device-resident solve", kMaxPast);
    REQUIRE(ctx, ctx->nranks == 1 || ctx->x_active, "the device-resident solve needs the in-kernel exchange (comm_p2p) when sharded");
    REQUIRE(ctx, B == 1 || ldx >= s->n, "solver_minimize: the batch stride of x is shorter than n");
    REQUIRE(ctx, trace_host == nullptr || B == 1, "solver_minimize: traces are recorded for single problems only");
    const bool coupled = objective == LBFGS_B200_OBJ_ROSENBROCK_CHAINED || objective == LBFGS_B200_OBJ_QUAD_TRIDIAG;
    if (objective == LBFGS_B200_OBJ_ROSENBROCK_PAIRED) REQUIRE(ctx, s->n % 2 == 0, "paired Rosenbrock needs an even n");
    if (objective == LBFGS_B200_OBJ_QUAD_TRIDIAG) REQUIRE(ctx, data0 && data1, "quad_tridiag needs data0 = diag, data1 = rhs");
    int64_t n_global = s->n, index_offset = ctx->index_offset;
    if (ctx->nranks > 1 && coupled)
    {
        REQUIRE(ctx, ctx->n_global > 0, "a neighbour-coupled objective under n-sharding needs lbfgs_b200_set_global_extent()");
        REQUIRE(ctx, ctx->index_offset + s->n <= ctx->n_global, "local block exceeds the global extent");
        REQUIRE(ctx, ctx->rank == ctx->nranks - 1 || s->n % 4 == 0, "every block but the last must hold a multiple of 4 coordinates");
        n_global = ctx->n_global;
    }
    else if (coupled) index_offset = 0;
    if (ctx->x_active) REQUIRE(ctx, (size_t)B * (s->pstride + 4) <= (size_t)kXMaxVals, "batch of %d problems with m = %d exceeds the exchange buffer", B, s->m);
    const int rounds = (s->m + kGramMaxWarps - 1) / kGramMaxWarps;
    void* kernel = persist_kernel_for<T>(objective, rounds);
    if (!kernel) return fail(ctx, LBFGS_B200_ERR_INVALID, "unknown objective id %d", objective);

    if (trace_host && trace_cap > s->trace_cap)
    {
        pool_free(ctx, s->d_trace);
        s->d_trace = nullptr;
        CU(ctx, pool_alloc(ctx, (void**)&s->d_trace, sizeof(double) * (size_t)trace_cap));
        s->trace_cap = trace_cap;
    }

    s->h_state.assign(sizeof(PState<T>) * (size_t)B, 0);
    PState<T>* hs = reinterpret_cast<PState<T>*>(s->h_state.data());
    const size_t vb = sizeof(T) * (size_t)s->n;
    for (int b = 0; b < B; b++)
    {
        PState<T>& p = hs[b];
        T* base = static_cast<T*>(s->vec_slab) + (size_t)b * 7 * s->vec_elems;
        p.x = base; p.xp = base + s->vec_elems; p.g = base + 2 * s->vec_elems; p.gp = base + 3 * s->vec_elems;
        p.drt = base + 4 * s->vec_elems; p.x_lo = base + 5 * s->vec_elems; p.g_lo = base + 6 * s->vec_elems;
        p.hist.H = static_cast<T*>(s->d_hist) + (size_t)b * s->hist_elems;
        p.hist.bt_log = s->bt_log; p.hist.M = s->M; p.hist.bstride = (int64_t)s->M * 2 * ((int64_t)1 << s->bt_log);
        T* small = static_cast<T*>(s->d_small) + (size_t)b * s->small_elems;
        const size_t mm = (size_t)s->M * s->M;
        p.ys = small; p.alpha = small + s->M; p.theta = small + 2 * s->M;
        for (int k = 0; k < 2; k++) { p.SY[k] = small + 2 * s->M + 4 + (3 * k + 0) * mm; p.YY[k] = small + 2 * s->M + 4 + (3 * k + 1) * mm; p.SS[k] = small + 2 * s->M + 4 + (3 * k + 2) * mm; }
        p.data0 = data0 ? data0 + (size_t)b * ldd : nullptr;
        p.data1 = data1 ? data1 + (size_t)b * ldd : nullptr;
        p.raw = s->d_raw + (size_t)b * s->pstride;
        p.halo = s->d_halo + (size_t)b * kHaloDoubles;
        p.head = 0; p.ncorr = 0; p.M = s->M; p.m = s->m; p.gram_cur = 0; p.pending = -1;
        p.op = POP_FIRST; p.c_round = 0;
        p.epsilon = (T)prm->epsilon; p.epsilon_rel = (T)prm->epsilon_rel; p.delta = (T)prm->delta; p.max_step = (T)prm->max_step;
        p.eps_gate = std::numeric_limits<T>::epsilon();
        p.past = prm->past; p.max_iterations = prm->max_iterations; p.ls_kind = ls_kind;
        p.fuse_first_trial = (coupled && ctx->nranks > 1) ? 0 : 1;
        p.adaptive_first_store = (getenv("LBFGS_B200_VIRTUAL_FIRST_TRIAL") && atoi(getenv("LBFGS_B200_VIRTUAL_FIRST_TRIAL")) != 0) ? 1 : 0;
        p.first_store = p.adaptive_first_store ? 0 : 1;
        p.ls_opt.linesearch = (ls_kind == 3) ? 3 : prm->linesearch;
        p.ls_opt.max_linesearch = prm->max_linesearch;
        p.ls_opt.min_step = (T)prm->min_step; p.ls_opt.max_step = (T)prm->max_step; p.ls_opt.ftol = (T)prm->ftol; p.ls_opt.wolfe = (T)prm->wolfe;
        p.trace = trace_host ? s->d_trace : nullptr;
        p.trace_cap = trace_host ? trace_cap : 0;
        CU(ctx, cudaMemcpyAsync(p.x, x_inout + (size_t)b * ldx, vb, cudaMemcpyDeviceToDevice, ctx->stream));
    }
    s->h_rounds.assign(sizeof(PRound<T>) * (size_t)B, 0);
    PRound<T>* hr = reinterpret_cast<PRound<T>*>(s->h_rounds.data());
    for (int b = 0; b < B; b++)
    {
        const PState<T>& p = hs[b];
        hr[b].x = p.x; hr[b].xp = p.xp; hr[b].g = p.g; hr[b].gp = p.gp; hr[b].drt = p.drt;
        hr[b].step = T(0); hr[b].op = p.op; hr[b].c_round = 0; hr[b].head = 0; hr[b].pending = -1; hr[b].gram_cur = p.gram_cur; hr[b].store_first = p.first_store;
    }
    CU(ctx, cudaMemsetAsync(s->d_small, 0, sizeof(T) * s->small_elems * (size_t)B, ctx->stream));
    {
        static const T one = T(1);
        for (int b = 0; b < B; b++) CU(ctx, cudaMemcpyAsync(hs[b].theta, &one, sizeof(T), cudaMemcpyHostToDevice, ctx->stream));
    }
    CU(ctx, cudaMemcpyAsync(s->d_state, hs, sizeof(PState<T>) * (size_t)B, cudaMemcpyHostToDevice, ctx->stream));
    CU(ctx, cudaMemcpyAsync(s->d_rounds, hr, sizeof(PRound<T>) * (size_t)B, cudaMemcpyHostToDevice, ctx->stream));
    PCtl hc{};
    hc.nactive = B;
    hc.epoch = ctx->x_epoch;
    CU(ctx, cudaMemcpyAsync(s->d_ctl, &hc, sizeof(hc), cudaMemcpyHostToDevice, ctx->stream));
    CU(ctx, cudaMemsetAsync(s->d_halo, 0, sizeof(double) * kHaloDoubles * (size_t)B, ctx->stream));

    const int64_t units = (s->n + ((int64_t)1 << s->bt_log) - 1) >> s->bt_log;
    const int grid = (int)(units < ctx->sm_count ? (units < 1 ? 1 : units) : ctx->sm_count);
    const size_t smem = (size_t)kPStageBytes;
    CU(ctx, cudaFuncSetAttribute(kernel, cudaFuncAttributeMaxDynamicSharedMemorySize, (int)smem));
    int per_sm = 0;
    CU(ctx, cudaOccupancyMaxActiveBlocksPerMultiprocessor(&per_sm, kernel, kPThreads, smem));
    REQUIRE(ctx, per_sm >= 1, "the persistent solve kernel does not fit on an SM of this device");
    PArgs<T> a{};
    a.probs = static_cast<PState<T>*>(s->d_state); a.rounds = static_cast<PRound<T>*>(s->d_rounds); a.B = B; a.ctl = s->d_ctl; a.partials = s->d_partials; a.pstride = s->pstride;
    a.n = s->n; a.grain = 1 << s->bt_log; a.xc = ctx->x_active ? ctx->x_comm : nullptr;
    a.index_offset = index_offset; a.n_global = n_global;
    a.wait_cycles = kPWaitCycles;
    if (const char* e = getenv("LBFGS_B200_WATCHDOG_SCALE")) { const long long k = atoll(e); if (k >= 1 && k <= 100000) a.wait_cycles *= k; }
    a.tune = ((size_t)s->n * sizeof(T) * 4 > ((size_t)96 << 20)) ? 4 : 0;
    if (const char* e = getenv("LBFGS_B200_TUNE")) a.tune = atoi(e);
    void* kargs[] = {&a};
    CU(ctx, cudaEventRecord(s->ev0, ctx->stream));
    CU(ctx, cudaLaunchCooperativeKernel(kernel, dim3((unsigned)grid), dim3(kPThreads), kargs, smem, ctx->stream));
    CU(ctx, cudaEventRecord(s->ev1, ctx->stream));
    ctx->launches++;
    CU(ctx, cudaMemcpyAsync(hs, s->d_state, sizeof(PState<T>) * (size_t)B, cudaMemcpyDeviceToHost, ctx->stream));
    CU(ctx, cudaMemcpyAsync(&hc, s->d_ctl, sizeof(hc), cudaMemcpyDeviceToHost, ctx->stream));
    CU(ctx, cudaStreamSynchronize(ctx->stream));
    ctx->x_epoch = hc.epoch;
    s->last_ctl = hc;
    CU(ctx, cudaEventElapsedTime(&s->last_kernel_ms, s->ev0, s->ev1));
    if (hc.abort) return fail(ctx, LBFGS_B200_ERR_CUDA, "the persistent solve gave up waiting at a grid / cross-rank barrier after %llu rounds (watchdog)", hc.rounds);

    for (int b = 0; b < B; b++)
    {
        const PState<T>& p = hs[b];
        CU(ctx, cudaMemcpyAsync(x_inout + (size_t)b * ldx, p.x, vb, cudaMemcpyDeviceToDevice, ctx->stream));
        s->final_g[b] = p.g;
        s->final_x[b] = p.x;
        s->ring_head[b] = p.head; s->ring_ncorr[b] = p.ncorr; s->ring_gram_cur[b] = p.gram_cur;
        s->export_fresh[b] = 0;
        outs[b].status = p.status;
        outs[b].niter = p.niter;
        outs[b].nfev = p.nfev;
        outs[b].fx = (double)p.fx;
        outs[b].gnorm = (double)p.gnorm;
        outs[b].rounds = p.rounds;
    }
    if (trace_host)
    {
        const long long cnt = hs[0].nfev < trace_cap ? hs[0].nfev : trace_cap;
        CU(ctx, cudaMemcpyAsync(trace_host, s->d_trace, sizeof(double) * (size_t)cnt, cudaMemcpyDeviceToHost, ctx->stream));
    }
    CU(ctx, cudaStreamSynchronize(ctx->stream));
    return LBFGS_B200_OK;
}

template <class T> __global__ void k_untile_history(lb::PHist<T> h, int64_t n, int64_t ld, T* __restrict__ S, T* __restrict__ Y)
{
    const int slot = blockIdx.y;
    for (int64_t i = (int64_t)blockIdx.x * blockDim.x + threadIdx.x; i < n; i += (int64_t)gridDim.x * blockDim.x)
    {
        S[(int64_t)slot * ld + i] = *h.s_at(slot, i);
        Y[(int64_t)slot * ld + i] = *h.y_at(slot, i);
    }
}
#if defined(LBFGS_B200_PERSIST_F64)
template <class T> static lbfgs_b200_hist* export_history(lbfgs_b200_solver* s, int b)
{
    lbfgs_b200_ctx* ctx = s->ctx;
    lbfgs_b200_hist*& h = s->exported[(size_t)b];
    if (h && s->export_fresh[(size_t)b]) return h;
    if (!h && lbfgs_b200_hist_create(ctx, &h, s->n, s->m, s->elem) != LBFGS_B200_OK) return nullptr;
    lb::PHist<T> ph;
    ph.H = static_cast<T*>(s->d_hist) + (size_t)b * s->hist_elems;
    ph.bt_log = s->bt_log; ph.M = s->M; ph.bstride = (int64_t)s->M * 2 * ((int64_t)1 << s->bt_log);
    const dim3 grid((unsigned)std::min<int64_t>((s->n + 255) / 256, 4 * ctx->sm_count), (unsigned)s->M);
    k_untile_history<T><<<grid, 256, 0, ctx->stream>>>(ph, s->n, h->ld, static_cast<T*>(h->S), static_cast<T*>(h->Y));
    const T* small = static_cast<const T*>(s->d_small) + (size_t)b * s->small_elems;
    const size_t mm = (size_t)s->M * s->M;
    cudaMemcpyAsync(h->ys, small, sizeof(T) * s->M, cudaMemcpyDeviceToDevice, ctx->stream);
    cudaMemcpyAsync(h->alpha, small + s->M, sizeof(T) * s->M, cudaMemcpyDeviceToDevice, ctx->stream);
    cudaMemcpyAsync(h->theta, small + 2 * s->M, sizeof(T), cudaMemcpyDeviceToDevice, ctx->stream);
    for (int k = 0; k < 2; k++)
    {
        cudaMemcpyAsync(h->SY[k], small + 2 * s->M + 4 + (3 * k + 0) * mm, sizeof(T) * mm, cudaMemcpyDeviceToDevice, ctx->stream);
        cudaMemcpyAsync(h->YY[k], small + 2 * s->M + 4 + (3 * k + 1) * mm, sizeof(T) * mm, cudaMemcpyDeviceToDevice, ctx->stream);
        cudaMemcpyAsync(h->SS[k], small + 2 * s->M + 4 + (3 * k + 2) * mm, sizeof(T) * mm, cudaMemcpyDeviceToDevice, ctx->stream);
    }
    if (cudaStreamSynchronize(ctx->stream) != cudaSuccess || cudaGetLastError() != cudaSuccess) { fail(ctx, LBFGS_B200_ERR_CUDA, "exporting the solver's history failed"); return nullptr; }
    h->head = s->ring_head[(size_t)b]; h->ncorr = s->ring_ncorr[(size_t)b]; h->gram_cur = s->ring_gram_cur[(size_t)b]; h->pending = -1;
    s->export_fresh[(size_t)b] = 1;
    return h;
}
#endif

extern "C" {

#ifdef LBFGS_B200_PERSIST_F64
lbfgs_b200_status lbfgs_b200_solver_create_batch(lbfgs_b200_ctx* ctx, int64_t n, int m, int elem_bytes, int batch, lbfgs_b200_solver** out)
{
    REQUIRE(ctx, ctx && out, "solver_create: NULL argument");
    *out = nullptr;
    REQUIRE(ctx, batch >= 1 && batch <= 4096, "solver_create: 1 <= batch <= 4096 (got %d)", batch);
    REQUIRE(ctx, n >= 1 && m >= 1 && m <= 64, "solver_create: need n >= 1 and 1 <= m <= 64 (got n=%lld m=%d)", (long long)n, m);
    REQUIRE(ctx, elem_bytes == 8 || elem_bytes == 4, "solver_create: elem_bytes must be 8 or 4");
    lbfgs_b200_solver* s = new (std::nothrow) lbfgs_b200_solver();
    if (!s) return fail(ctx, LBFGS_B200_ERR_ALLOC, "out of host memory");
    s->ctx = ctx; s->n = n; s->m = m; s->elem = elem_bytes; s->B = batch;
    s->final_g.assign((size_t)batch, nullptr);
    s->final_x.assign((size_t)batch, nullptr);
    s->M = m + 1;
    {
        int bt = 1024, want_stages = 2;
        if (const char* e = getenv("LBFGS_B200_STAGES")) { const int v = atoi(e); if (v >= 1 && v <= lb::kPMaxStages) want_stages = v; }
        while (bt > 32 && (size_t)want_stages * (2 * m + 4) * bt * elem_bytes > (size_t)lb::kPStageBytes) bt >>= 1;
        s->bt_log = 0;
        while ((1 << s->bt_log) < bt) s->bt_log++;
    }
    const int64_t nblocks = (n + ((int64_t)1 << s->bt_log) - 1) >> s->bt_log;
    s->hist_elems = (size_t)nblocks * s->M * 2 * ((size_t)1 << s->bt_log);
    s->small_elems = (size_t)2 * s->M + 4 + 6 * (size_t)s->M * s->M;
    s->ring_head.assign((size_t)batch, 0); s->ring_ncorr.assign((size_t)batch, 0); s->ring_gram_cur.assign((size_t)batch, 0);
    s->exported.assign((size_t)batch, nullptr); s->export_fresh.assign((size_t)batch, 0);
    cudaError_t e = cudaSuccess;
    s->vec_elems = (((size_t)n * elem_bytes + 255) & ~size_t(255)) / elem_bytes;
    s->pstride = ((m * lb::kGramVals > 8 ? m * lb::kGramVals : 8) + 7) & ~7;
    const size_t state_bytes = (elem_bytes == 8 ? sizeof(lb::PState<double>) : sizeof(lb::PState<float>)) * (size_t)batch;
    if (e == cudaSuccess) e = pool_alloc(ctx, (void**)&s->vec_slab, (size_t)batch * 7 * s->vec_elems * elem_bytes);
    if (e == cudaSuccess) e = pool_alloc(ctx, (void**)&s->d_hist, (size_t)batch * s->hist_elems * elem_bytes);
    if (e == cudaSuccess) e = pool_alloc(ctx, (void**)&s->d_small, (size_t)batch * s->small_elems * elem_bytes);
    if (e == cudaSuccess) e = pool_alloc(ctx, (void**)&s->d_state, state_bytes);
    if (e == cudaSuccess) e = pool_alloc(ctx, (void**)&s->d_rounds, (elem_bytes == 8 ? sizeof(lb::PRound<double>) : sizeof(lb::PRound<float>)) * (size_t)batch);
    if (e == cudaSuccess) e = pool_alloc(ctx, (void**)&s->d_ctl, sizeof(lb::PCtl));
    if (e == cudaSuccess) e = pool_alloc(ctx, (void**)&s->d_partials, sizeof(double) * (size_t)batch * s->pstride * ctx->sm_count);
    if (e == cudaSuccess) e = pool_alloc(ctx, (void**)&s->d_raw, sizeof(double) * (size_t)batch * s->pstride);
    if (e == cudaSuccess) e = pool_alloc(ctx, (void**)&s->d_halo, sizeof(double) * (size_t)batch * lb::kHaloDoubles);
    if (e == cudaSuccess) e = cudaEventCreate(&s->ev0);
    if (e == cudaSuccess) e = cudaEventCreate(&s->ev1);
    if (e != cudaSuccess)
    {
        lbfgs_b200_solver_destroy(s);
        return fail(ctx, e == cudaErrorMemoryAllocation ? LBFGS_B200_ERR_ALLOC : LBFGS_B200_ERR_CUDA, "solver_create: %s", cudaGetErrorString(e));
    }
    *out = s;
    return LBFGS_B200_OK;
}

lbfgs_b200_status lbfgs_b200_solver_create(lbfgs_b200_ctx* ctx, int64_t n, int m, int elem_bytes, lbfgs_b200_solver** out)
{
    return lbfgs_b200_solver_create_batch(ctx, n, m, elem_bytes, 1, out);
}

void lbfgs_b200_solver_destroy(lbfgs_b200_solver* s)
{
    if (!s) return;
    if (s->ctx && s->ctx->stream) cudaStreamSynchronize(s->ctx->stream);
    for (void* p : {(void*)s->vec_slab, (void*)s->d_state, (void*)s->d_rounds, (void*)s->d_ctl, (void*)s->d_partials, (void*)s->d_raw, (void*)s->d_halo,
                    (void*)s->d_trace, (void*)s->d_hist, (void*)s->d_small})
        pool_free(s->ctx, p);
    if (s->ev0) cudaEventDestroy(s->ev0);
    if (s->ev1) cudaEventDestroy(s->ev1);
    for (lbfgs_b200_hist* h : s->exported) lbfgs_b200_hist_destroy(h);
    delete s;
}

int lbfgs_b200_solver_batch(const lbfgs_b200_solver* s) { return s ? s->B : 0; }
lbfgs_b200_status lbfgs_b200_solver_profile(const lbfgs_b200_solver* s, double* kernel_ms, double* ms_by_op10, unsigned long long* rounds_by_op10,
                                            double* alg_bytes_by_op10, double* sync_ms)
{
    if (!s) return LBFGS_B200_ERR_INVALID;
    const lb::PCtl& c = s->last_ctl;
    long long total = 0;
    for (int k = 0; k < lb::kPOps; k++) total += c.cyc_op[k];
    const double scale = total > 0 ? (double)s->last_kernel_ms / (double)total : 0.0;
    if (kernel_ms) *kernel_ms = s->last_kernel_ms;
    for (int k = 0; k < lb::kPOps; k++)
    {
        if (ms_by_op10) ms_by_op10[k] = scale * (double)c.cyc_op[k];
        if (rounds_by_op10) rounds_by_op10[k] = c.n_op[k];
        if (alg_bytes_by_op10) alg_bytes_by_op10[k] = c.words_op[k] * (double)s->n * (double)s->elem;
    }
    if (sync_ms) { sync_ms[0] = scale * (double)c.cyc_sync; sync_ms[1] = scale * (double)c.cyc_wait_all; sync_ms[2] = scale * (double)c.cyc_exchange; }
    return LBFGS_B200_OK;
}
const void* lbfgs_b200_solver_final_grad(const lbfgs_b200_solver* s) { return s ? s->final_g[0] : nullptr; }
const void* lbfgs_b200_solver_final_grad_of(const lbfgs_b200_solver* s, int b) { return (s && b >= 0 && b < s->B) ? s->final_g[(size_t)b] : nullptr; }
lbfgs_b200_hist* lbfgs_b200_solver_history_of(lbfgs_b200_solver* s, int b)
{
    if (!s || b < 0 || b >= s->B) return nullptr;
    if (s->elem == 8) return export_history<double>(s, b);
    return export_history<float>(s, b);
}
lbfgs_b200_hist* lbfgs_b200_solver_history(lbfgs_b200_solver* s) { return lbfgs_b200_solver_history_of(s, 0); }

lbfgs_b200_status lbfgs_b200_solver_minimize_f64(lbfgs_b200_solver* s, int objective, const double* data0, const double* data1,
                                                 const lbfgs_b200_param* prm, int line_search, double* x_inout, double* trace_host,
                                                 long long trace_cap, lbfgs_b200_outcome* out)
{
    if (!s || !s->ctx) return LBFGS_B200_ERR_INVALID;
    if (s->B != 1) return fail(s->ctx, LBFGS_B200_ERR_INVALID, "solver_minimize: the solver holds a batch of %d problems, use solver_minimize_batch", s->B);
    return solver_minimize<double>(s, objective, data0, data1, 0, prm, line_search, x_inout, s->n, trace_host, trace_cap, out);
}
lbfgs_b200_status lbfgs_b200_solver_minimize_batch_f64(lbfgs_b200_solver* s, int objective, const double* data0, const double* data1, int64_t ldd,
                                                       const lbfgs_b200_param* prm, int line_search, double* x_inout, int64_t ldx,
                                                       lbfgs_b200_outcome* outs)
{
    if (!s || !s->ctx) return LBFGS_B200_ERR_INVALID;
    return solver_minimize<double>(s, objective, data0, data1, ldd, prm, line_search, x_inout, ldx, nullptr, 0, outs);
}
#endif

#ifdef LBFGS_B200_PERSIST_F32
lbfgs_b200_status lbfgs_b200_solver_minimize_f32(lbfgs_b200_solver* s, int objective, const float* data0, const float* data1,
                                                 const lbfgs_b200_param* prm, int line_search, float* x_inout, double* trace_host,
                                                 long long trace_cap, lbfgs_b200_outcome* out)
{
    if (!s || !s->ctx) return LBFGS_B200_ERR_INVALID;
    if (s->B != 1) return fail(s->ctx, LBFGS_B200_ERR_INVALID, "solver_minimize: the solver holds a batch of %d problems, use solver_minimize_batch", s->B);
    return solver_minimize<float>(s, objective, data0, data1, 0, prm, line_search, x_inout, s->n, trace_host, trace_cap, out);
}
lbfgs_b200_status lbfgs_b200_solver_minimize_batch_f32(lbfgs_b200_solver* s, int objective, const float* data0, const float* data1, int64_t ldd,
                                                       const lbfgs_b200_param* prm, int line_search, float* x_inout, int64_t ldx,
                                                       lbfgs_b200_outcome* outs)
{
    if (!s || !s->ctx) return LBFGS_B200_ERR_INVALID;
    return solver_minimize<float>(s, objective, data0, data1, ldd, prm, line_search, x_inout, ldx, nullptr, 0, outs);
}

#endif

}
```

Measured before the change: 1566.

## Speculatively fuse next-iteration pair dots into the first-trial combine pass

```diff
diff --git a/lbfgspp_b200/csrc/device_utils.cuh b/lbfgspp_b200/csrc/device_utils.cuh
--- a/lbfgspp_b200/csrc/device_utils.cuh
+++ b/lbfgspp_b200/csrc/device_utils.cuh
@@ -79,7 +79,7 @@
 
 constexpr int kXMaxRanks = 8;
 constexpr int kXRing = 4;
-constexpr int kXMaxVals = 4608;
+constexpr int kXMaxVals = 5120;
 constexpr int kMailVals = 384;
 
 struct XInbox
diff --git a/lbfgspp_b200/csrc/persist.cuh b/lbfgspp_b200/csrc/persist.cuh
--- a/lbfgspp_b200/csrc/persist.cuh
+++ b/lbfgspp_b200/csrc/persist.cuh
@@ -5,11 +5,13 @@
 namespace lb {
 
 constexpr int kMaxPast = 64;
-constexpr int kPThreads = kGramMaxThreads;
+constexpr int kPThreads = 512;
 constexpr int kPWarps = kPThreads / 32;
 constexpr int kPStageBytes = kGramStages * 4 * kGramTE * 8;
 constexpr int kPMaxStages = 4;
 constexpr int kPCache = 4;
+constexpr int kSpecDefault = 1;
+constexpr int kDotsCols = 5;
 
 enum { POP_IDLE = 0, POP_FIRST = 1, POP_TRIAL = 2, POP_DOTS_FORM = 3, POP_DOTS_PLAIN = 4, POP_COMBINE = 5, POP_COMBINE_TRIAL = 6, POP_RESTORE = 7,
        POP_MATERIALIZE = 8 };
@@ -51,6 +53,9 @@
     int lo_virtual;
     T lo_step;
     int after_materialize;
+    int spec_policy;
+    int spec_now;
+    int last_first_accepted;
     T fx, dg, gg, xx, gnorm, step;
     int k;
     long long nfev;
@@ -67,7 +72,7 @@
 {
     T *x, *xp, *g, *gp, *drt;
     T step;
-    int op, c_round, head, pending, gram_cur, store_first;
+    int op, c_round, head, pending, gram_cur, store_first, spec;
 };
 
 struct alignas(128) PCtl
@@ -165,7 +170,7 @@
 struct PShared
 {
     uint64_t full_bar[kPMaxStages];
-    double red[kPWarps][3 * kGramVals];
+    double red[kPWarps][kDotsCols * kGramVals];
     double coef[2 * kMaxM + 2];
     const void* vecs[2 * kMaxM + 2];
     unsigned char slots[kMaxM];
@@ -452,24 +457,106 @@
     else if (tid == nrhs + 1 && bbytes) tma_load_1d(dstt + (size_t)(nrhs + 2 * (runs.a1 - runs.a0)) * TE, blk + (size_t)runs.b0 * 2 * TE, bbytes, bar);
 }
 
+struct DotsMap
+{
+    int units, cpg;
+    int u, q, j0, ncols;
+    __device__ __forceinline__ DotsMap(int units_, int c) : units(units_)
+    {
+        const int groups = kPThreads / units > 1 ? kPThreads / units : 1;
+        cpg = (c + groups - 1) / groups;
+        u = threadIdx.x % units;
+        q = threadIdx.x / units;
+        j0 = q * cpg;
+        ncols = (q < groups && c > j0) ? (c - j0 < cpg ? c - j0 : cpg) : 0;
+    }
+};
+
+template <class T, bool FORM>
+__device__ __forceinline__ void dots_unit(T (&acc)[kDotsCols][kGramVals], Unit<T> ug, Unit<T> usn, Unit<T> uyn, int cnt, const T* hist, int TE, int off,
+                                          const DotsMap& dm, const unsigned char* rows)
+{
+    constexpr int EPT = 16 / (int)sizeof(T);
+    if (cnt < EPT)
+    {
+        mask_unit(ug, cnt);
+        if (FORM) { mask_unit(usn, cnt); mask_unit(uyn, cnt); }
+    }
+#pragma unroll
+    for (int i = 0; i < kDotsCols; i++)
+    {
+        if (i >= dm.ncols) break;
+        const int j = dm.j0 + i;
+        Unit<T> us, uy;
+        if (FORM && j == 0) { us = usn; uy = uyn; }
+        else
+        {
+            const T* srow = hist + (size_t)2 * rows[FORM ? j - 1 : j] * TE;
+            us = lds_unit<T>(srow + off);
+            uy = lds_unit<T>(srow + TE + off);
+            if (cnt < EPT) { mask_unit(us, cnt); mask_unit(uy, cnt); }
+        }
+#pragma unroll
+        for (int k = 0; k < EPT; k++)
+        {
+            acc[i][0] += us.v[k] * ug.v[k];
+            acc[i][1] += uy.v[k] * ug.v[k];
+        }
+        if constexpr (FORM)
+        {
+#pragma unroll
+            for (int k = 0; k < EPT; k++)
+            {
+                acc[i][2] += us.v[k] * uyn.v[k];
+                acc[i][3] += uy.v[k] * uyn.v[k];
+                acc[i][4] += uy.v[k] * usn.v[k];
+                acc[i][5] += us.v[k] * usn.v[k];
+            }
+        }
+    }
+}
+
+template <class T>
+__device__ __forceinline__ void dots_reduce(const T (&acc)[kDotsCols][kGramVals], const DotsMap& dm, int c, PShared& sh, double* dst, int G)
+{
+    const int tid = threadIdx.x, lane = tid & 31, warp = tid >> 5;
+    __syncthreads();
+#pragma unroll
+    for (int i = 0; i < kDotsCols; i++)
+#pragma unroll
+        for (int k = 0; k < kGramVals; k++)
+        {
+            const double w = warp_sum((double)acc[i][k]);
+            if (lane == 0) sh.red[warp][i * kGramVals + k] = w;
+        }
+    __syncthreads();
+    const int wpg = dm.units / 32;
+    for (int idx = tid; idx < c * kGramVals; idx += kPThreads)
+    {
+        const int j = idx / kGramVals, k = idx % kGramVals;
+        const int q = j / dm.cpg, i = j % dm.cpg;
+        double t = 0.0;
+        for (int w = q * wpg; w < (q + 1) * wpg; w++) t += sh.red[w][i * kGramVals + k];
+        dst[(size_t)idx * G] = t;
+    }
+}
+
 template <class T> struct PDots
 {
     int64_t n;
     PHist<T> h;
     int c;
     int end, cnt_old;
-    int new_slot, split, cols_per_round;
+    int new_slot;
 };
 
-template <class T, int ROUNDS, bool FORM>
+template <class T, bool FORM>
 __device__ __forceinline__ void p_dots(const PDots<T>& a, const Own& own, T* tiles, PShared& sh, unsigned& phase_bits, double* dst, int G)
 {
     constexpr int EPT = 16 / (int)sizeof(T);
     constexpr int NRHS = FORM ? 4 : 1;
-    const int tid = threadIdx.x, lane = tid & 31, warp = tid >> 5;
     const int TE = a.h.BT();
-    const int my_col = warp / a.split, my_part = warp % a.split;
-    const int upp = (TE / EPT) / a.split;
+    const DotsMap dm(TE / EPT, a.c);
     const SlotRuns runs(a.end, a.cnt_old, a.h.M);
     const int nrows = NRHS + 2 * a.cnt_old;
     int stages = (int)((size_t)kPStageBytes / ((size_t)nrows * TE * sizeof(T)));
@@ -477,80 +564,41 @@
     const int64_t ntl = own.ntiles(TE);
     uint64_t* full_bar = sh.full_bar;
 
-    T acc[ROUNDS][kGramVals];
-#pragma unroll
-    for (int r = 0; r < ROUNDS; r++)
-#pragma unroll
-        for (int k = 0; k < kGramVals; k++) acc[r][k] = T(0);
+    T acc[kDotsCols][kGramVals];
+#pragma unroll
+    for (int i = 0; i < kDotsCols; i++)
+#pragma unroll
+        for (int k = 0; k < kGramVals; k++) acc[i][k] = T(0);
 
     __syncthreads();
     int64_t next_tile = 0;
     for (int s = 0; s < stages; s++, next_tile++)
         if (next_tile < ntl) stage_tiled<T>(tiles + (size_t)s * nrows * TE, TE, NRHS, own.start(next_tile, TE), own.len(next_tile, TE), a.h, runs, sh, &full_bar[s]);
     int stage = 0;
+    const int off = dm.u * EPT;
     for (int64_t t = 0; t < ntl; t++)
     {
         mbar_wait(&full_bar[stage], (phase_bits >> stage) & 1u);
         phase_bits ^= (1u << stage);
         const T* base = tiles + (size_t)stage * nrows * TE;
-        const T* hist = base + (size_t)NRHS * TE;
-        const int64_t e0 = own.start(t, TE);
-        const int len = own.len(t, TE);
-#pragma unroll
-        for (int r = 0; r < ROUNDS; r++)
-        {
-            const int j = r * a.cols_per_round + my_col;
-            if (my_col < a.cols_per_round && j < a.c)
-            {
-                const bool is_new = FORM && j == 0;
-                const T* srow = hist + (size_t)2 * (is_new ? 0 : sh.slots[j]) * TE;
-                const T* yrow = srow + TE;
-                T* s_new = a.h.s_at(a.new_slot < 0 ? 0 : a.new_slot, e0);
-                for (int u = my_part * upp + lane; u < (my_part + 1) * upp; u += 32)
+        const int cnt = own.len(t, TE) - off;
+        if (dm.ncols > 0 && cnt > 0)
+        {
+            const Unit<T> ug = lds_unit<T>(base + off);
+            Unit<T> usn{}, uyn{};
+            if constexpr (FORM)
+            {
+                const Unit<T> ux = lds_unit<T>(base + TE + off), ugp = lds_unit<T>(base + 2 * TE + off), uxp = lds_unit<T>(base + 3 * TE + off);
+#pragma unroll
+                for (int k = 0; k < EPT; k++) { usn.v[k] = ux.v[k] - uxp.v[k]; uyn.v[k] = ug.v[k] - ugp.v[k]; }
+                if (dm.q == 0)
                 {
-                    const int off = u * EPT;
-                    const int cnt = len - off;
-                    if (cnt <= 0) break;
-                    Unit<T> ug = lds_unit<T>(base + off), us, uy, usn, uyn;
-                    if constexpr (FORM)
-                    {
-                        const Unit<T> ux = lds_unit<T>(base + TE + off), ugp = lds_unit<T>(base + 2 * TE + off), uxp = lds_unit<T>(base + 3 * TE + off);
-#pragma unroll
-                        for (int k = 0; k < EPT; k++) { usn.v[k] = ux.v[k] - uxp.v[k]; uyn.v[k] = ug.v[k] - ugp.v[k]; }
-                        if (cnt < EPT) { mask_unit(usn, cnt); mask_unit(uyn, cnt); }
-                    }
-                    bool loaded = false;
-                    if constexpr (FORM)
-                    {
-                        if (is_new)
-                        {
-                            us = usn; uy = uyn;
-                            st_unit<T>(s_new, off, cnt, usn);
-                            st_unit<T>(s_new + TE, off, cnt, uyn);
-                            loaded = true;
-                        }
-                    }
-                    if (!loaded) { us = lds_unit<T>(srow + off); uy = lds_unit<T>(yrow + off); }
-                    if (cnt < EPT) { mask_unit(ug, cnt); mask_unit(us, cnt); mask_unit(uy, cnt); }
-#pragma unroll
-                    for (int k = 0; k < EPT; k++)
-                    {
-                        acc[r][0] += us.v[k] * ug.v[k];
-                        acc[r][1] += uy.v[k] * ug.v[k];
-                    }
-                    if constexpr (FORM)
-                    {
-#pragma unroll
-                        for (int k = 0; k < EPT; k++)
-                        {
-                            acc[r][2] += us.v[k] * uyn.v[k];
-                            acc[r][3] += uy.v[k] * uyn.v[k];
-                            acc[r][4] += uy.v[k] * usn.v[k];
-                            acc[r][5] += us.v[k] * usn.v[k];
-                        }
-                    }
+                    T* s_new = a.h.s_at(a.new_slot, own.start(t, TE));
+                    st_unit<T>(s_new, off, cnt, usn);
+                    st_unit<T>(s_new + TE, off, cnt, uyn);
                 }
             }
+            dots_unit<T, FORM>(acc, ug, usn, uyn, cnt, base + (size_t)NRHS * TE, TE, off, dm, sh.slots);
         }
         asm volatile("fence.proxy.async.shared::cta;" ::: "memory");
         __syncthreads();
@@ -558,48 +606,24 @@
         next_tile++;
         stage = (stage + 1 == stages) ? 0 : stage + 1;
     }
-
-#pragma unroll
-    for (int r = 0; r < ROUNDS; r++)
-#pragma unroll
-        for (int k = 0; k < kGramVals; k++)
-        {
-            const double w = warp_sum((double)acc[r][k]);
-            if (lane == 0) sh.red[warp][r * kGramVals + k] = w;
-        }
-    __syncthreads();
-    const int nvals = a.c * kGramVals;
-    for (int idx = tid; idx < nvals; idx += kPThreads)
-    {
-        const int j = idx / kGramVals, k = idx % kGramVals;
-        const int r = j / a.cols_per_round, col = j % a.cols_per_round;
-        double t = 0.0;
-        for (int p = 0; p < a.split; p++) t += sh.red[col * a.split + p][r * kGramVals + k];
-        dst[(size_t)idx * G] = t;
-    }
-}
-
-__device__ __forceinline__ void dots_geometry(int c, int units, int& split, int& cols_per_round)
-{
-    split = 8;
-    while (split > 1 && (c * split > kGramMaxWarps || units / split < 32)) split >>= 1;
-    cols_per_round = c < kGramMaxWarps / split ? c : kGramMaxWarps / split;
-}
-
-template <class T, class OBJ, bool FUSE, bool HALO, class Between>
+    dots_reduce<T>(acc, dm, a.c, sh, dst, G);
+}
+
+template <class T, class OBJ, bool FUSE, bool HALO, bool SPEC, class Between>
 __device__ __forceinline__ void p_combine(const OBJ& obj, const Own& own, const PHist<T>& h, int c, int end, T* tiles, T* __restrict__ res,
                                           T* __restrict__ x1_out, T* __restrict__ g1_out, PShared& sh, unsigned& phase_bits, double* dst, int G,
-                                          Between between)
+                                          int spec_c, int new_slot, Between between)
 {
     constexpr int EPT = 16 / (int)sizeof(T);
     constexpr int DV = HALO ? OBJ::kDataVectors : 0;
     constexpr int NRHS = (FUSE ? 2 : 1) + DV;
     constexpr int PAD = EPT;
+    static_assert(!SPEC || (FUSE && !HALO), "speculative pair dots ride on the fused first trial of a non-coupled objective");
     const int tid = threadIdx.x, lane = tid & 31, warp = tid >> 5;
     const int TE = h.BT();
     const SlotRuns runs(end, c, h.M);
     const int nrows = NRHS + 2 * c;
-    const size_t stage_elems = (size_t)nrows * TE + (HALO ? 2 * PAD : 0);
+    const size_t stage_elems = (size_t)(nrows + (SPEC ? 1 : 0)) * TE + (HALO ? 2 * PAD : 0);
     int stages = (int)((size_t)kPStageBytes / (stage_elems * sizeof(T)));
     stages = stages > kPMaxStages ? kPMaxStages : stages;
     const int64_t n = own.n;
@@ -632,6 +656,12 @@
 
     T acc[5] = {T(0), T(0), T(0), T(0), T(0)};
     T pre[5] = {T(0), T(0), T(0), T(0), T(0)};
+    const DotsMap dm(TE / EPT, spec_c);
+    T accd[kDotsCols][kGramVals];
+#pragma unroll
+    for (int i = 0; i < kDotsCols; i++)
+#pragma unroll
+        for (int k = 0; k < kGramVals; k++) accd[i][k] = T(0);
     __syncthreads();
     int64_t next_tile = 0;
     for (int s = 0; s < stages; s++, next_tile++)
@@ -708,7 +738,27 @@
                         st_unit<T>(x1_out, i0, cnt, uo);
                         st_unit<T>(g1_out, i0, cnt, ug);
                     }
+                    if constexpr (SPEC)
+                    {
+                        Unit<T> usn, uyn;
+#pragma unroll
+                        for (int k = 0; k < EPT; k++) { usn.v[k] = uo.v[k] - ux.v[k]; uyn.v[k] = ug.v[k] - uv.v[k]; }
+                        *reinterpret_cast<float4*>(base + (size_t)nrows * TE + off) = *reinterpret_cast<const float4*>(ug.v);
+                        *reinterpret_cast<float4*>(xrow + off) = *reinterpret_cast<const float4*>(usn.v);
+                        *reinterpret_cast<float4*>(base + off) = *reinterpret_cast<const float4*>(uyn.v);
+                        T* s_new = h.s_at(new_slot, e0);
+                        st_unit<T>(s_new, off, cnt, usn);
+                        st_unit<T>(s_new + TE, off, cnt, uyn);
+                    }
                 }
+            }
+            if constexpr (SPEC)
+            {
+                __syncthreads();
+                const int off = dm.u * EPT, cnt = len - off;
+                if (dm.ncols > 0 && cnt > 0)
+                    dots_unit<T, true>(accd, lds_unit<T>(base + (size_t)nrows * TE + off), lds_unit<T>(xrow + off), lds_unit<T>(base + off), cnt, hist, TE, off,
+                                       dm, sh.slots);
             }
         }
         else
@@ -820,8 +870,14 @@
     }
     if (FUSE)
     {
+        double* dst_trial = dst;
+        if constexpr (SPEC)
+        {
+            dots_reduce<T>(accd, dm, spec_c, sh, dst, G);
+            dst_trial = dst + (size_t)spec_c * kGramVals * G;
+        }
         const double dacc[5] = {(double)acc[0], (double)acc[1], (double)acc[2], (double)acc[3], (double)acc[4]};
-        block_sums<5>(dacc, sh, dst, G);
+        block_sums<5>(dacc, sh, dst_trial, G);
     }
     else
     {
@@ -890,6 +946,7 @@
     const T step_tried = ls_step_ref(st);
     const int rc = ls_advance(st, fx, dg, keep);
     if (is_first && st->adaptive_first_store) st->first_store = (rc == LBFGSpp::LSC_ACCEPT) ? 1 : 0;
+    if (is_first) st->last_first_accepted = (rc == LBFGSpp::LSC_ACCEPT) ? 1 : 0;
     if (keep)
     {
         if (is_virtual) { st->lo_virtual = 1; st->lo_step = step_tried; }
@@ -950,7 +1007,32 @@
     return true;
 }
 
-template <class T> __device__ void advance_problem(PState<T>* st, const double* vals)
+template <class T> __device__ __forceinline__ int dots_form_columns(const PState<T>* st) { return st->ncorr < st->m ? st->ncorr + 1 : st->m; }
+
+template <class T> __device__ __forceinline__ void schedule_combine(PState<T>* st, bool can_spec)
+{
+    st->op = st->fuse_first_trial ? POP_COMBINE_TRIAL : POP_COMBINE;
+    const bool want = st->spec_policy == 1 || (st->spec_policy == 2 && st->last_first_accepted);
+    st->spec_now = (can_spec && want && st->fuse_first_trial && st->first_store) ? 1 : 0;
+}
+
+template <class T> __device__ __forceinline__ void after_pair_dots(PState<T>* st, const double* vals, bool can_spec)
+{
+    const T sy = (T)vals[2], yy = (T)vals[3];
+    if (sy > st->eps_gate * yy)
+    {
+        st->ys[st->head] = sy;
+        *st->theta = yy / sy;
+        st->pending = st->head;
+        st->head = (st->head + 1) % st->M;
+        st->ncorr = st->c_round;
+        schedule_combine(st, can_spec);
+    }
+    else if (st->ncorr > 0) { st->op = POP_DOTS_PLAIN; st->c_round = st->ncorr; }
+    else { st->c_round = 0; schedule_combine(st, can_spec); }
+}
+
+template <class T> __device__ void advance_problem(PState<T>* st, const double* vals, bool can_spec)
 {
     st->rounds++;
     switch (st->op)
@@ -977,41 +1059,35 @@
         after_search(st);
         return;
     case POP_DOTS_FORM:
-    {
-        const T sy = (T)vals[2], yy = (T)vals[3];
-        if (sy > st->eps_gate * yy)
-        {
-            st->ys[st->head] = sy;
-            *st->theta = yy / sy;
-            st->pending = st->head;
-            st->head = (st->head + 1) % st->M;
-            st->ncorr = st->c_round;
-            st->op = st->fuse_first_trial ? POP_COMBINE_TRIAL : POP_COMBINE;
-        }
-        else if (st->ncorr > 0) { st->op = POP_DOTS_PLAIN; st->c_round = st->ncorr; }
-        else { st->op = st->fuse_first_trial ? POP_COMBINE_TRIAL : POP_COMBINE; st->c_round = 0; }
+        after_pair_dots(st, vals, can_spec);
         return;
-    }
     case POP_DOTS_PLAIN:
-        st->op = st->fuse_first_trial ? POP_COMBINE_TRIAL : POP_COMBINE;
+        schedule_combine(st, can_spec);
         return;
     case POP_COMBINE:
     case POP_COMBINE_TRIAL:
     {
         const bool fused = st->op == POP_COMBINE_TRIAL;
         const bool stored = st->first_store != 0;
+        const bool spec = fused && st->spec_now != 0;
+        const double* tv = vals + (spec ? dots_form_columns(st) * kGramVals : 0);
+        st->spec_now = 0;
         if (st->pending >= 0) { st->gram_cur = 1 - st->gram_cur; st->pending = -1; }
-        st->dg = (T)vals[0];
+        st->dg = (T)tv[0];
         st->k += 1;
         if (!begin_search(st, T(1))) return;
-        if (fused && ls_step_ref(st) == T(1)) digest_trial(st, (T)vals[1], (T)vals[2], (T)vals[3], (T)vals[4], true, !stored);
+        if (fused && ls_step_ref(st) == T(1))
+        {
+            digest_trial(st, (T)tv[1], (T)tv[2], (T)tv[3], (T)tv[4], true, !stored);
+            if (spec && st->op == POP_DOTS_FORM) after_pair_dots(st, vals, can_spec);
+        }
         return;
     }
     default: return;
     }
 }
 
-__device__ __forceinline__ double words_of(int op, int c, int data_vectors, int store_first)
+__device__ __forceinline__ double words_of(int op, int c, int data_vectors, int store_first, int spec)
 {
     switch (op)
     {
@@ -1021,7 +1097,7 @@
     case POP_DOTS_FORM: return 2.0 * c + 4.0;
     case POP_DOTS_PLAIN: return 2.0 * c + 1.0;
     case POP_COMBINE: return 2.0 * c + 2.0;
-    case POP_COMBINE_TRIAL: return 2.0 * c + 3.0 + (store_first ? 2.0 : 0.0) + data_vectors;
+    case POP_COMBINE_TRIAL: return 2.0 * c + 3.0 + (store_first ? 2.0 : 0.0) + (spec ? 2.0 : 0.0) + data_vectors;
     default: return 0.0;
     }
 }
@@ -1033,7 +1109,7 @@
     case POP_FIRST: case POP_TRIAL: case POP_MATERIALIZE: return 4;
     case POP_DOTS_FORM: case POP_DOTS_PLAIN: return st->c_round * kGramVals;
     case POP_COMBINE: return 1;
-    case POP_COMBINE_TRIAL: return 5;
+    case POP_COMBINE_TRIAL: return 5 + (st->spec_now ? dots_form_columns(st) * kGramVals : 0);
     default: return 0;
     }
 }
@@ -1142,12 +1218,13 @@
         if (b < a.B && state_of(b)->op != POP_IDLE)
         {
             PState<T>* st = state_of(b);
-            advance_problem(st, st->raw);
+            advance_problem(st, st->raw, !HALO);
             PRound<T>* rd = a.rounds + b;
             rd->x = st->x; rd->xp = st->xp; rd->g = st->g; rd->gp = st->gp; rd->drt = st->drt;
             rd->step = st->step;
             rd->c_round = st->c_round; rd->head = st->head; rd->pending = st->pending; rd->gram_cur = st->gram_cur;
             rd->store_first = st->first_store;
+            rd->spec = st->spec_now;
             rd->op = st->op;
             running = st->op != POP_IDLE;
         }
@@ -1196,7 +1273,7 @@
     if (tid == 0) a.ctl->epoch = epoch;
 }
 
-template <class T, class OBJ, int ROUNDS>
+template <class T, class OBJ>
 __global__ void __launch_bounds__(kPThreads, 1) k_persist(PArgs<T> a)
 {
     extern __shared__ __align__(128) unsigned char p_smem[];
@@ -1293,9 +1370,10 @@
             const T step = ldv(&rd->step);
             const int c_round = ldv(&rd->c_round), head = ldv(&rd->head), pending = ldv(&rd->pending), gram_cur = ldv(&rd->gram_cur);
             const int store_first = ldv(&rd->store_first);
+            const int spec = ldv(&rd->spec);
             if (op == POP_IDLE) continue;
             acct_bucket = (acct_bucket == -1 || acct_bucket == op) ? op : 0;
-            acct_words += words_of(op, c_round, kDataVectors, store_first);
+            acct_words += words_of(op, c_round, kDataVectors, store_first, op == POP_COMBINE_TRIAL ? spec : 0);
             double* dst = a.partials + (size_t)b * a.pstride * G + cta;
             const OBJ obj = PObjMaker<T, OBJ>::make(a, st->data0, st->data1, (HALO && a.xc != nullptr) ? st->halo : nullptr);
             switch (op)
@@ -1321,16 +1399,14 @@
                 d.end = head;
                 d.cnt_old = form ? c_round - 1 : c_round;
                 d.new_slot = form ? head : -1;
-                dots_geometry(d.c, d.h.BT() / (16 / (int)sizeof(T)), d.split, d.cols_per_round);
                 __syncthreads();
                 {
                     const SlotRuns runs(d.end, d.cnt_old, d.h.M);
-                    if (tid < d.c && !(form && tid == 0))
-                        sh.slots[tid] = (unsigned char)runs.row_of(slot_by_age(head, d.h.M, form ? tid - 1 : tid));
+                    if (tid < d.cnt_old) sh.slots[tid] = (unsigned char)runs.row_of(slot_by_age(head, d.h.M, tid));
                     if (tid == 0) { sh.vecs[0] = vg; sh.vecs[1] = vx; sh.vecs[2] = vgp; sh.vecs[3] = vxp; }
                 }
-                if (form) p_dots<T, ROUNDS, true>(d, own, tiles, sh, phase_bits, dst, G);
-                else p_dots<T, ROUNDS, false>(d, own, tiles, sh, phase_bits, dst, G);
+                if (form) p_dots<T, true>(d, own, tiles, sh, phase_bits, dst, G);
+                else p_dots<T, false>(d, own, tiles, sh, phase_bits, dst, G);
                 break;
             }
             case POP_COMBINE:
@@ -1367,8 +1443,17 @@
                 };
                 if (!own_scratch) solve_into(tiles);
                 auto between = [&]() { if (own_scratch) solve_into(reinterpret_cast<T*>(s_gram)); };
-                if (fuse) p_combine<T, OBJ, true, OBJ::kHalo>(obj, own, st->hist, g.c, head, tiles, vd, store_first ? vxp : nullptr, store_first ? vgp : nullptr, sh, phase_bits, dst, G, between);
-                else p_combine<T, OBJ, false, false>(obj, own, st->hist, g.c, head, tiles, vd, nullptr, nullptr, sh, phase_bits, dst, G, between);
+                const int spec_c = g.c + 1 < st->m ? g.c + 1 : st->m;
+                bool done = false;
+                if constexpr (!HALO)
+                    if (fuse && spec && store_first)
+                    {
+                        p_combine<T, OBJ, true, false, true>(obj, own, st->hist, g.c, head, tiles, vd, vxp, vgp, sh, phase_bits, dst, G, spec_c, head, between);
+                        done = true;
+                    }
+                if (done) {}
+                else if (fuse) p_combine<T, OBJ, true, OBJ::kHalo, false>(obj, own, st->hist, g.c, head, tiles, vd, store_first ? vxp : nullptr, store_first ? vgp : nullptr, sh, phase_bits, dst, G, 0, -1, between);
+                else p_combine<T, OBJ, false, false, false>(obj, own, st->hist, g.c, head, tiles, vd, nullptr, nullptr, sh, phase_bits, dst, G, 0, -1, between);
                 break;
             }
             default: break;
diff --git a/lbfgspp_b200/csrc/persist_host.cuh b/lbfgspp_b200/csrc/persist_host.cuh
--- a/lbfgspp_b200/csrc/persist_host.cuh
+++ b/lbfgspp_b200/csrc/persist_host.cuh
@@ -32,10 +32,10 @@
     lb::PCtl last_ctl{};
 };
 
-template <class T> static void* persist_kernel_for(int objective, int rounds)
+template <class T> static void* persist_kernel_for(int objective)
 {
     using namespace lb;
-#define LB_PK(OBJ) (rounds <= 1 ? (void*)k_persist<T, OBJ, 1> : rounds == 2 ? (void*)k_persist<T, OBJ, 2> : (void*)k_persist<T, OBJ, 3>)
+#define LB_PK(OBJ) ((void*)k_persist<T, OBJ>)
     switch (objective)
     {
     case LBFGS_B200_OBJ_ROSENBROCK_PAIRED: return LB_PK(RosenbrockPaired<T>);
@@ -75,8 +75,7 @@
     }
     else if (coupled) index_offset = 0;
     if (ctx->x_active) REQUIRE(ctx, (size_t)B * (s->pstride + 4) <= (size_t)kXMaxVals, "batch of %d problems with m = %d exceeds the exchange buffer", B, s->m);
-    const int rounds = (s->m + kGramMaxWarps - 1) / kGramMaxWarps;
-    void* kernel = persist_kernel_for<T>(objective, rounds);
+    void* kernel = persist_kernel_for<T>(objective);
     if (!kernel) return fail(ctx, LBFGS_B200_ERR_INVALID, "unknown objective id %d", objective);
 
     if (trace_host && trace_cap > s->trace_cap)
@@ -114,6 +113,9 @@
         p.fuse_first_trial = (coupled && ctx->nranks > 1) ? 0 : 1;
         p.adaptive_first_store = (getenv("LBFGS_B200_VIRTUAL_FIRST_TRIAL") && atoi(getenv("LBFGS_B200_VIRTUAL_FIRST_TRIAL")) != 0) ? 1 : 0;
         p.first_store = p.adaptive_first_store ? 0 : 1;
+        p.spec_policy = coupled ? 0 : kSpecDefault;
+        if (const char* e = getenv("LBFGS_B200_SPECULATE")) { const int v = atoi(e); if (v >= 0 && v <= 2 && !coupled) p.spec_policy = v; }
+        p.spec_now = 0; p.last_first_accepted = 0;
         p.ls_opt.linesearch = (ls_kind == 3) ? 3 : prm->linesearch;
         p.ls_opt.max_linesearch = prm->max_linesearch;
         p.ls_opt.min_step = (T)prm->min_step; p.ls_opt.max_step = (T)prm->max_step; p.ls_opt.ftol = (T)prm->ftol; p.ls_opt.wolfe = (T)prm->wolfe;
@@ -127,7 +129,7 @@
     {
         const PState<T>& p = hs[b];
         hr[b].x = p.x; hr[b].xp = p.xp; hr[b].g = p.g; hr[b].gp = p.gp; hr[b].drt = p.drt;
-        hr[b].step = T(0); hr[b].op = p.op; hr[b].c_round = 0; hr[b].head = 0; hr[b].pending = -1; hr[b].gram_cur = p.gram_cur; hr[b].store_first = p.first_store;
+        hr[b].step = T(0); hr[b].op = p.op; hr[b].c_round = 0; hr[b].head = 0; hr[b].pending = -1; hr[b].gram_cur = p.gram_cur; hr[b].store_first = p.first_store; hr[b].spec = 0;
     }
     CU(ctx, cudaMemsetAsync(s->d_small, 0, sizeof(T) * s->small_elems * (size_t)B, ctx->stream));
     {
@@ -252,7 +254,9 @@
     {
         int bt = 1024, want_stages = 2;
         if (const char* e = getenv("LBFGS_B200_STAGES")) { const int v = atoi(e); if (v >= 1 && v <= lb::kPMaxStages) want_stages = v; }
-        while (bt > 32 && (size_t)want_stages * (2 * m + 4) * bt * elem_bytes > (size_t)lb::kPStageBytes) bt >>= 1;
+        const int ept = 16 / elem_bytes;
+        auto cols_per_group = [&](int b) { const int groups = std::max(1, lb::kPThreads / (b / ept)); return (m + groups - 1) / groups; };
+        while (bt > 32 * ept && ((size_t)want_stages * (2 * m + 4) * bt * elem_bytes > (size_t)lb::kPStageBytes || cols_per_group(bt) > lb::kDotsCols)) bt >>= 1;
         s->bt_log = 0;
         while ((1 << s->bt_log) < bt) s->bt_log++;
     }
@@ -263,7 +267,7 @@
     s->exported.assign((size_t)batch, nullptr); s->export_fresh.assign((size_t)batch, 0);
     cudaError_t e = cudaSuccess;
     s->vec_elems = (((size_t)n * elem_bytes + 255) & ~size_t(255)) / elem_bytes;
-    s->pstride = ((m * lb::kGramVals > 8 ? m * lb::kGramVals : 8) + 7) & ~7;
+    s->pstride = (m * lb::kGramVals + 5 + 7) & ~7;
     const size_t state_bytes = (elem_bytes == 8 ? sizeof(lb::PState<double>) : sizeof(lb::PState<float>)) * (size_t)batch;
     if (e == cudaSuccess) e = pool_alloc(ctx, (void**)&s->vec_slab, (size_t)batch * 7 * s->vec_elems * elem_bytes);
     if (e == cudaSuccess) e = pool_alloc(ctx, (void**)&s->d_hist, (size_t)batch * s->hist_elems * elem_bytes);
```

Result: faster. 1884 (median of 6 runs) (+20.3%).
